# ihmcrobotics/mecano

Measured on AMD Instinct MI355X. Metric: robot-configs/sec (RNEA+ABA), 30-DoF humanoid batch=4096, higher is better.
Workload: dtype f64; 1 GPU; 30-DoF humanoid (SixDoF pelvis + 24 revolute), RNEA and ABA of every configuration per step, fp64, AoS [B][n] state; entry_point=mh_rnea_aba_f64, batch_per_gpu=4096, global_batch=4096, nq=31, nv=30, bodies=25, parallelism=dp1 (batch sharded, no data-path collective), kernel_variant=topo:b5c1e26c784c54fa, model_seed=43, state_seed=2342

## Files before the change

### mecano_amd/csrc/mh_api.hip

```cpp
#include "../../include/mecano_hip.h"
#include "mh_dfs_kernels.h"
#include "mh_split_kernels.h"
#include "mh_gravity_kernels.h"
#include "mh_response_kernels.h"
#include "mh_minv_kernels.h"

#include <dlfcn.h>
#include <spawn.h>
#include <sys/wait.h>
#include <unistd.h>
#include <cerrno>
extern char **environ;
#include <unistd.h>

#include <algorithm>
#include <functional>
#include <array>
#include <cmath>
#include <cstdarg>
#include <cstdio>
#include <cstdlib>
#include <cstring>
#include <map>
#include <deque>
// ... 332 lines not shown
   d.consts = sizeof(T) == 8 ? (const void *)m->d_consts64 : (const void *)m->d_consts32;
   d.prog = m->d_prog, d.n_events = (int)m->prog.size();
   d.rnea_stack = m->rnea_stack, d.aba_stack = m->aba_stack, d.aba_hand = m->aba_hand;
   return d;
}

template <class ARGS>
void set_root_acceleration(ARGS &A, const mh_options &o, const double *gravity)
{
   using T = decltype(A.gx);
   if (o.use_root_acceleration)
   {
      A.rax = (T)o.root_acceleration[0], A.ray = (T)o.root_acceleration[1], A.raz = (T)o.root_acceleration[2];
      A.gx = (T)-o.root_acceleration[3], A.gy = (T)-o.root_acceleration[4], A.gz = (T)-o.root_acceleration[5];
   }
   else
   {
      A.rax = T(0), A.ray = T(0), A.raz = T(0);
      A.gx = gravity ? (T)gravity[0] : T(0), A.gy = gravity ? (T)gravity[1] : T(0), A.gz = gravity ? (T)gravity[2] : T(0);
   }
}

mh_status check_common(mh_model_t &model, int64_t B, const mh_options *opts)
{
   if (!model)
      return fail(MH_ERR_INVALID_ARGUMENT, "model is NULL");
   if (opts && opts->context)
   {
      mh_model *c = ((mh_context *)opts->context)->m;
      if (c->parent != (model->parent ? model->parent : model))
         return fail(MH_ERR_INVALID_ARGUMENT, "opts->context belongs to another model");
      model = c;
   }
   if (B < 0)
      return fail(MH_ERR_BAD_DIMENSION, "negative batch size %lld", (long long)B);
   if (opts && opts->layout != MH_LAYOUT_AOS && opts->layout != MH_LAYOUT_SOA)
      return fail(MH_ERR_INVALID_ARGUMENT, "unknown layout %d", opts->layout);
   int cur = 0;
   if (hipGetDevice(&cur) != hipSuccess)
      return fail(MH_ERR_NO_DEVICE, "no usable HIP device");
   if (cur != model->device)
      return fail(MH_ERR_INVALID_ARGUMENT, "model lives on device %d but the calling thread's device is %d", model->device, cur);
   return MH_OK;
}
mh_status begin_call(mh_model_t &model, int64_t B, const mh_options *opts_in, mh_options &opts)
{
   if (opts_in)
      opts = *opts_in;
   else
      mh_options_default(&opts);
   return check_common(model, B, &opts);
}

long groups_of(int64_t B) { return (B + 63) / 64; }

void set_strides(long &bs, long &es, bool soa, int64_t B, long n) { bs = soa ? 1 : n, es = soa ? B : 1; }

template <typename T>
mh::Args<T> make_args(const mh_model *m, int64_t B, const mh_options &o)
{
   mh::Args<T> A{};
   A.m = dev_model<T>(m);
   A.B = B;
   const bool soa = o.layout == MH_LAYOUT_SOA;
   set_strides(A.q_bs, A.q_es, soa, B, m->nq);
   set_strides(A.v_bs, A.v_es, soa, B, m->nv);
   set_strides(A.f_bs, A.f_es, soa, B, (long)m->n * 6);
   return A;
}
template <typename T>
mh::Args<T> make_args(const mh_model *m, int64_t B, const mh_options &o, const double *gravity)
{
   mh::Args<T> A = make_args<T>(m, B, o);
   set_root_acceleration(A, o, gravity);
   A.coriolis = o.consider_coriolis, A.accel = o.consider_accelerations;
   return A;
}

bool spec_done(int rc, const char *what, mh_status &st)
{
   if (rc == (int)hipErrorNotSupported)
      return false;
   st = rc == 0 ? MH_OK : fail(MH_ERR_HIP, "%s: %s", what, hipGetErrorString((hipError_t)rc));
   return true;
}

mh_status raise_lds_limit(mh_model *model, const void *kern, size_t lds)
{
   if (lds > 64 * 1024 && model->lds_attr[kern] < lds)
   {
      HIP_TRY(hipFuncSetAttribute(kern, hipFuncAttributeMaxDynamicSharedMemorySize, (int)lds));
      model->lds_attr[kern] = lds;
   }
   return MH_OK;
}

bool auto_transpose(const mh_model *m, int64_t B) { return B >= 8192 && m->nq + m->nv >= 64; }
bool transposes(const mh_model *m, int64_t B) { return m->use_transpose >= 0 ? m->use_transpose != 0 : auto_transpose(m, B); }

int split_flags(const mh_model *m, int algo, bool soa)
{
   int flags = m->ident_maps ? SPEC_IDENT : 0;
   if (!soa && m->dense_maps && m->force_io != 0 && m->spec.split_lds_bytes(algo, SPEC_IO_LDS, m->nq, m->nv) <= 160 * 1024)
      flags |= SPEC_IO_LDS;
   return flags;
}
bool split_ok(const mh_model *m, int algo, int64_t B, bool soa)
{
   if (!m->spec.launch_split || !m->spec.split_usable || !m->spec.split_usable() || !m->use_spec || m->use_split == 0)
      return false;
   if (m->spec.split_lds_bytes(algo, split_flags(m, algo, soa), m->nq, m->nv) > 160 * 1024)
      return false;
   if (m->use_split == 1 || algo == 1 || algo == 0)
      return true;
   const long groups = groups_of(B);
   const long waves = groups * 4 * (algo == 2 ? 2 : 1);
   return waves <= (long)m->cu_count * 4 * kFusedFactor;
}

bool zv_ok(const mh_model *m, int64_t B, bool soa, int jobs)
{
   if (!m->spec.launch_zv || !m->spec.zv_usable || !m->spec.zv_usable() || !m->use_spec || !m->use_zv || m->use_split == 0)
      return false;
   if (soa || !m->dense_maps || m->force_io == 0 || m->n_locked > 0)
      return false;
   const long lds = m->spec.zv_lds_bytes(m->nq, m->nv);
   return lds > 0 && lds <= 160 * 1024 && (m->use_zv == 2 || groups_of(B) * jobs <= (long)m->cu_count);
}
std::mutex g_error_words_mutex;
std::vector<int *> g_error_words;
mh_status zv_check_error(mh_model *m)
{
   if (m->zv_error_host && *(volatile int *)m->zv_error_host != 0)
   {
      *(volatile int *)m->zv_error_host = 0;
      return fail(MH_ERR_HIP, "a bias-split forward dynamics launch gave up waiting for its bias rows (the accelerations of those configurations were written as NaN)");
   }
   return MH_OK;
}
mh_status check_all_error_words()
{
   std::lock_guard<std::mutex> lock(g_error_words_mutex);
   bool any = false;
   for (int *w : g_error_words)
      if (*(volatile int *)w != 0)
      {
         *(volatile int *)w = 0;
         any = true;
      }
   if (any)
      return fail(MH_ERR_HIP, "a bias-split forward dynamics launch gave up waiting for its bias rows (the accelerations of those configurations were written as NaN)");
   return MH_OK;
}
bool zv_self_signalling(const mh_model *m) { return m->ident_maps && m->spec.zv_self_signal && m->spec.zv_self_signal() != 0; }
mh_status zv_prepare(mh_model *m, int64_t B, hipStream_t stream)
{
   const size_t groups = (size_t)groups_of(B);
   mh_status st = ensure_bytes(m->zv_tau, groups * 64 * m->nv * sizeof(double));
   if (st != MH_OK)
      return st;
   if (zv_self_signalling(m) && m->zv_cols.bytes < groups * 64 * m->nv * sizeof(double))
   {
      st = ensure_bytes(m->zv_cols, std::max<size_t>(groups, 128) * 64 * m->nv * sizeof(double));
      if (st != MH_OK)
         return st;
      HIP_TRY(hipMemsetD32Async((hipDeviceptr_t)m->zv_cols.ptr, 0x7ff4a5a5, m->zv_cols.bytes / 4, stream));
   }
   if (m->zv_flags.bytes < groups * mh::ZV_SYNC_STRIDE * sizeof(int))
   {
      st = ensure_bytes(m->zv_flags, std::max<size_t>(groups, 1024) * mh::ZV_SYNC_STRIDE * sizeof(int));
      if (st != MH_OK)
         return st;
      HIP_TRY(hipMemsetAsync(m->zv_flags.ptr, 0, m->zv_flags.bytes, stream));
      m->zv_epoch = 0;
   }
   if (!m->zv_error_host)
   {
      HIP_TRY(hipHostMalloc((void **)&m->zv_error_host, 2 * sizeof(int), hipHostMallocMapped));
      m->zv_error_host[0] = m->zv_error_host[1] = 0;
      HIP_TRY(hipHostGetDevicePointer((void **)&m->zv_error_dev, m->zv_error_host, 0));
      std::lock_guard<std::mutex> lock(g_error_words_mutex);
      g_error_words.push_back(m->zv_error_host);
   }
   return MH_OK;
}
mh_status zv_launch(mh_model *m, mh::Args<double> &A, int jobs, hipStream_t stream, bool &done)
{
   done = false;
   mh_status st = zv_prepare(m, A.B, stream);
   if (st != MH_OK)
      return st;
   if (m->zv_epoch == 0x7fffffff)
   {
      HIP_TRY(hipDeviceSynchronize());
      HIP_TRY(hipMemsetAsync(m->zv_flags.ptr, 0, m->zv_flags.bytes, stream));
      m->zv_epoch = 0;
   }
   const bool self_signal = zv_self_signalling(m);
   if (self_signal && *(volatile int *)(m->zv_error_host + 1) != 0)
   {
      HIP_TRY(hipDeviceSynchronize());
      HIP_TRY(hipMemsetD32Async((hipDeviceptr_t)m->zv_cols.ptr, 0x7ff4a5a5, m->zv_cols.bytes / 4, stream));
      HIP_TRY(hipMemsetAsync(m->zv_flags.ptr, 0, m->zv_flags.bytes, stream));
      m->zv_epoch = 0;
      *(volatile int *)(m->zv_error_host + 1) = 0;
   }
   const int epoch = ++m->zv_epoch;
   int flags = SPEC_IO_LDS | (m->ident_maps ? SPEC_IDENT : 0);
   done = spec_done(m->spec.launch_zv(flags, &A, self_signal ? m->zv_cols.ptr : m->zv_tau.ptr, (int *)m->zv_flags.ptr, m->zv_error_dev, epoch, jobs,
                                      m->zv_same_l2, m->zv_wait_ticks, (void *)stream),
                    "bias-split kernel launch failed", st);
   return st;
}

bool zvb_ok(const mh_model *m, int64_t B, bool soa)
{
   if (!m->spec.launch_zvb || !m->spec.zvb_usable || !m->spec.zvb_usable() || !m->use_spec || !m->use_zvb || m->use_split == 0)
      return false;
   if (soa || !m->dense_maps || m->force_io == 0 || m->n_locked > 0)
      return false;
   return m->use_zvb == 2 || groups_of(B) >= 2 * (long)m->cu_count;
}
bool zvf_ok(const mh_model *m, int64_t B, bool soa)
{
   if (!m->spec.launch_zvf || !m->spec.zvf_usable || !m->spec.zvf_usable() || !m->use_spec || !m->use_zvf || m->use_split == 0)
      return false;
   if (soa || !m->dense_maps || !m->ident_maps || m->force_io == 0 || m->n_locked > 0)
      return false;
   return m->use_zvf == 2 || groups_of(B) > (long)m->cu_count;
}
bool rnea_ahead_ok(const mh_model *m, int64_t B, bool soa)
{
   if (!m->spec.launch_rnea_ahead || !m->spec.zvb_usable || !m->spec.zvb_usable() || !m->use_spec || !m->use_rnea_ahead || m->use_split == 0)
      return false;
   if (soa || !m->dense_maps || m->force_io == 0)
      return false;
   return m->use_rnea_ahead == 2 || groups_of(B) > 2 * (long)m->cu_count;
}
mh_status zvb_launch(mh_model *m, mh::Args<double> &A, hipStream_t stream, bool &done)
{
   done = false;
   const size_t padded = (size_t)(groups_of(A.B) * 64);
   mh_status st = ensure_bytes(m->zv_tau, (size_t)A.B * m->nv * sizeof(double));
   if (st == MH_OK)
      st = ensure_bytes(m->zvb_cs, std::max<size_t>(1, (size_t)m->spec.zvb_cs_rows()) * padded * sizeof(double));
   if (st != MH_OK)
      return st;
   const int flags = SPEC_IO_LDS | (m->ident_maps ? SPEC_IDENT : 0);
   const long groups = std::min<long>(groups_of(A.B), (long)m->cu_count * 2);
   done = spec_done(m->spec.launch_zvb(flags, &A, m->zv_tau.ptr, m->zvb_cs.ptr, (long)padded, (int)groups, m->zvb_which, (void *)stream),
                    "two-launch forward dynamics failed to launch", st);
   return st;
}

enum Algo
{
   ALGO_RNEA,
   ALGO_ABA,
   ALGO_CRBA
};

const mh_model::DfsPlan *dfs_plan(mh_model *m, int algo, int budget)
{
   if (m->parent)
      m = m->parent;
   std::lock_guard<std::mutex> lock(m->dfs_mutex);
   for (const mh_model::DfsPlan &p : m->dfs_plans)
      if (p.algo == algo && p.budget == budget)
         return &p;
   const int n = m->n;
   std::vector<int> meta = m->meta, frame(n), below(n, 0), lofs(n, 0), gofs(n, 0);
   std::vector<char> home(n, 0);
   auto MI = [&](int e, int k) -> int & { return meta[(size_t)e * mh::MI_STRIDE + k]; };
   for (int e = 0; e < n; e++)
      frame[e] = algo == 0 ? mh::rnea_frame_slots(MI(e, mh::MI_TYPE), MI(e, mh::MI_NCH))
                           : (algo == 1 ? mh::aba_frame_slots(MI(e, mh::MI_TYPE), MI(e, mh::MI_NCH)) : mh::pair_frame_slots(MI(e, mh::MI_TYPE), MI(e, mh::MI_NCH)));
   bool all_fit = true;
   {
      for (int e = n - 1; e >= 0; e--)
      {
         int need = below[e];
         if (frame[e] > 0 && below[e] + frame[e] <= budget)
            home[e] = 1, need += frame[e];
         else if (frame[e] > 0)
            all_fit = false;
         const int pe = MI(e, mh::MI_PARENT);
         if (pe >= 0)
            below[pe] = std::max(below[pe], need);
      }
   }
   if (!(m->dfs_place_greedy || (algo == 0 && budget < 64) || all_fit))
   {
      std::vector<int> worth(n, 0);
      std::vector<int> with_subtree(n, 0);
      for (int e = 0; e < n; e++)
         if (MI(e, mh::MI_PARENT) >= 0 && MI(e, mh::MI_NCH) > 0)
            with_subtree[MI(e, mh::MI_PARENT)]++;
      for (int e = 0; e < n; e++)
      {
         const int k = MI(e, mh::MI_NCH), jx = mh::jx_slots(MI(e, mh::MI_TYPE)), in_frame = std::max(0, with_subtree[e] - 1);
         if (k == 0)
            continue;
         if (algo == 0)
            worth[e] = k == 1 ? 2 * (6 + jx) : (6 + jx + 12) + (k - 1) * 12 + 6 + in_frame * 12 + (6 + jx);
         else
         {
            const int id = algo == 2 ? 6 : 0;
            const int acc = 27 + id;
            worth[e] = k == 1 ? 2 * (6 + jx) + 2 * id
                              : (12 + jx + 6 + id) + (k - 1) * (12 + id) + (in_frame > 0 ? acc + (in_frame - 1) * 2 * acc + acc : 0) + (12 + jx);
         }
      }
      const int W = budget + 1;
      std::vector<long> best((size_t)n * W, 0);
      std::vector<char> take((size_t)n * W, 0);
      std::vector<std::vector<int>> kids(n);
// ... 3309 lines not shown
```

### mecano_amd/csrc/mh_spec.hip

```cpp
#include "mh_spec_kernels.h"
#include "mh_zv_kernels.h"

#include <algorithm>
#include <atomic>
#include <cstdlib>
#include <type_traits>

#ifndef MH_SPEC_PART
#define MH_SPEC_PART 0
#endif
#ifndef MH_TOPO_N
#error "MH_TOPO_N / MH_TOPO_PARENTS / MH_TOPO_TYPES must be defined"
#endif

namespace
{
struct TP
{
   static constexpr int N = MH_TOPO_N;
   static constexpr int parent[N] = {MH_TOPO_PARENTS};
   static constexpr int type[N] = {MH_TOPO_TYPES};
};
constexpr int kParents[TP::N] = {MH_TOPO_PARENTS};
constexpr int kTypes[TP::N] = {MH_TOPO_TYPES};
// ... 73 lines not shown
      else
      {
         if (flags & F_ST_LDS)
            return go<ALGO, IO, ID, true>(A, grid, lds, s);
         return go<ALGO, IO, ID, false>(A, grid, lds, s);
      }
   }
   else
   {
      if constexpr (!kWholeTreeRnea)
         return hipErrorNotSupported;
      else
         return go<ALGO, IO, ID, false>(A, grid, lds, s);
   }
}
template <int ALGO>
hipError_t go_flags(int flags, const mh::Args<double> &A, int grid, size_t lds, hipStream_t s)
{
   const bool io = flags & F_IO_LDS, id = flags & F_IDENT;
   if (io && id)
      return go_st<ALGO, true, true>(flags, A, grid, lds, s);
   if (io)
      return go_st<ALGO, true, false>(flags, A, grid, lds, s);
   if (id)
      return go_st<ALGO, false, true>(flags, A, grid, lds, s);
   return go_st<ALGO, false, false>(flags, A, grid, lds, s);
}
}

template <bool ID>
hipError_t go_fused(const mh::Args<double> &A, int waves, hipStream_t stream)
{
   if constexpr (!kWholeTreeAba)
      return hipErrorNotSupported;
   else
   {
   auto kern = &mh::spec_fused_kernel<TP, double, ID>;
   const size_t lds = (size_t)std::max(lds_bytes(0, F_IO_LDS, A.m.nq, A.m.nv), lds_bytes(1, F_ST_LDS, A.m.nq, A.m.nv));
   static LdsAttr attr;
   if (const hipError_t e = ensure_lds_attr(reinterpret_cast<const void *>(kern), lds, attr); e != hipSuccess)
      return e;
   hipLaunchKernelGGL(kern, dim3(2 * waves), dim3(64), lds, stream, A);
   return hipGetLastError();
   }
}

using SPL = mh::Split<TP>;
static long split_lds_bytes(int algo, int flags, int nq, int nv)
{
   if (algo == 2)
      return std::max(split_lds_bytes(0, flags, nq, nv), split_lds_bytes(1, flags, nq, nv));
   long b = (long)(SPL::n_limbs() * (algo == 0 ? 6 : 27) + (algo == 1 ? SPL::TRUNK_SLOTS : SPL::RNEA_TRUNK_SLOTS)) * 64 * sizeof(double);
   if (flags & F_IO_LDS)
      b += (long)(nq + (algo == 1 ? 3 : 2) * nv) * 64 * sizeof(double);
   return b;
}
template <class K>
hipError_t launch_lds(K kern, const mh::Args<double> &A, int grid, size_t lds, LdsAttr &attr, hipStream_t stream)
{
   if (const hipError_t e = ensure_lds_attr(reinterpret_cast<const void *>(kern), lds, attr); e != hipSuccess)
      return e;
   hipLaunchKernelGGL(kern, dim3(grid), dim3(256), lds, stream, A);
   return hipGetLastError();
}
template <bool ID, bool IO>
hipError_t go_fused_split(const mh::Args<double> &A, int groups, hipStream_t stream)
{
   if constexpr (SPL::usable())
   {
      static LdsAttr attr_bytes;
      return launch_lds(&mh::spec_fused_split_kernel<TP, double, ID, IO>, A, 2 * groups,
                        (size_t)split_lds_bytes(2, IO ? F_IO_LDS : 0, A.m.nq, A.m.nv), attr_bytes, stream);
   }
   else
      return hipErrorNotSupported;
}
template <int ALGO, bool ID, bool IO>
hipError_t go_split(const mh::Args<double> &A, int groups, hipStream_t stream, bool occ3 = false)
{
   if constexpr (SPL::usable())
   {
      static LdsAttr attr_bytes, attr_occ3;
      if constexpr (ALGO == 0 && ID && !IO)
      {
         if (occ3)
            return launch_lds(&mh::spec_split_kernel_occ3<TP, double, ALGO, ID, IO>, A, groups,
                              (size_t)split_lds_bytes(ALGO, 0, A.m.nq, A.m.nv), attr_occ3, stream);
      }
      return launch_lds(&mh::spec_split_kernel<TP, double, ALGO, ID, IO>, A, groups,
                        (size_t)split_lds_bytes(ALGO, IO ? F_IO_LDS : 0, A.m.nq, A.m.nv), attr_bytes, stream);
   }
   else
      return hipErrorNotSupported;
}
template <bool ID, bool IO>
hipError_t go_split_algo(int algo, const mh::Args<double> &A, int groups, hipStream_t s, bool occ3)
{
   if (algo == 2)
      return go_fused_split<ID, IO>(A, groups, s);
   if (algo == 0)
      return go_split<0, ID, IO>(A, groups, s, occ3);
   if (algo == 1)
      return go_split<1, ID, IO>(A, groups, s);
   return hipErrorNotSupported;
}

extern "C" {
#if MH_SPEC_PART != 2
int mh_spec_split_usable(void) { return SPL::usable() ? 1 : 0; }
long mh_spec_split_lds_bytes(int algo, int flags, int nq, int nv) { return split_lds_bytes(algo, flags, nq, nv); }
int mh_spec_launch_split(int algo, int flags, const void *args, int groups, void *stream)
{
   const mh::Args<double> &A = *(const mh::Args<double> *)args;
   const bool id = flags & F_IDENT, io = flags & F_IO_LDS;
   hipStream_t s = (hipStream_t)stream;
   const bool occ3 = (flags & F_OCC3) != 0;
   if (flags & F_BODIES)
   {
#ifdef MH_SPEC_MINIMAL
      return (int)hipErrorNotSupported;
#else
      if constexpr (SPL::usable())
      {
         if (id && io && (algo == 0 || algo == 1))
         {
            static LdsAttr attr0, attr1;
            const size_t lds = (size_t)split_lds_bytes(algo, F_IO_LDS, A.m.nq, A.m.nv);
            if (algo == 0)
               return (int)launch_lds(&mh::spec_split_kernel<TP, double, 0, true, true, true>, A, groups, lds, attr0, s);
            return (int)launch_lds(&mh::spec_split_kernel<TP, double, 1, true, true, true>, A, groups, lds, attr1, s);
         }
      }
      return (int)hipErrorNotSupported;
#endif
   }
   if (id && io)
      return (int)go_split_algo<true, true>(algo, A, groups, s, occ3);
#ifdef MH_SPEC_MINIMAL
   return (int)hipErrorNotSupported;
#else
   if (id)
      return (int)go_split_algo<true, false>(algo, A, groups, s, occ3);
   if (io)
      return (int)go_split_algo<false, true>(algo, A, groups, s, occ3);
   return (int)go_split_algo<false, false>(algo, A, groups, s, occ3);
#endif
}
#endif
#if MH_SPEC_PART != 1
long mh_spec_zv_lds_bytes(int nq, int nv)
{
   if constexpr (!SPL::usable())
      return 0;
   const long inertia = (long)(SPL::n_limbs() * mh::ZV_XW + SPL::ZV_TRUNK_SLOTS + nq + 2 * nv) * 64 * (long)sizeof(double);
   return std::max(inertia, split_lds_bytes(0, F_IO_LDS, nq, nv) + (long)mh::zv_bias_extra_rows<TP>() * 64 * (long)sizeof(double));
}
int mh_spec_zv_usable(void) { return SPL::usable() ? 1 : 0; }
int mh_spec_zv_self_signal(void) { return MH_ZV_TWO_STAGE && MH_ZV_SELF_SIGNAL ? 1 : 0; }
#ifdef MH_ZV_PROBE
int mh_spec_zv_probe_read(void *dst, size_t bytes) { return (int)hipMemcpyFromSymbol(dst, HIP_SYMBOL(mh::zv_probe), bytes); }
int mh_spec_zv_probe_body_read(void *dst, size_t bytes) { return (int)hipMemcpyFromSymbol(dst, HIP_SYMBOL(mh::zv_probe_body), bytes); }
#endif
int mh_spec_launch_zv(int flags, const void *args, void *taup, int *sync_flags, int *error, int epoch, int jobs, int same_l2, unsigned wait_ticks, void *stream)
{
   if constexpr (SPL::usable())
   {
      const mh::Args<double> &A = *(const mh::Args<double> *)args;
      if (!(flags & F_IO_LDS) || (jobs != 2 && jobs != 3))
         return (int)hipErrorNotSupported;
      const size_t lds = (size_t)mh_spec_zv_lds_bytes(A.m.nq, A.m.nv);
      if (lds > 160 * 1024)
         return (int)hipErrorNotSupported;
      const long groups = (A.B + 63) / 64, padded = (groups + 7) / 8 * 8;
      const mh::ZvSync sy{sync_flags, error, epoch, jobs, same_l2 ? 1 : 0, wait_ticks};
      hipStream_t s = (hipStream_t)stream;
      if (A.q_next && (!(flags & F_IDENT) || jobs != 2 || !MH_ZV_TWO_STAGE))
         return (int)hipErrorNotSupported;
      if ((flags & F_IDENT) && A.q_next)
      {
         static LdsAttr attr_step;
         auto kern = &mh::spec_zv_kernel<TP, double, true, true>;
         if (const hipError_t e = ensure_lds_attr(reinterpret_cast<const void *>(kern), lds, attr_step); e != hipSuccess)
            return (int)e;
         hipLaunchKernelGGL(kern, dim3((unsigned)(padded * jobs)), dim3(256), lds, s, A.q, A.qd, A.in3b, A.B, jobs, A, (double *)taup, sy);
         return (int)hipGetLastError();
      }
      if (flags & F_IDENT)
      {
         static LdsAttr attr;
         auto kern = &mh::spec_zv_kernel<TP, double, true>;
         if (const hipError_t e = ensure_lds_attr(reinterpret_cast<const void *>(kern), lds, attr); e != hipSuccess)
            return (int)e;
         hipLaunchKernelGGL(kern, dim3((unsigned)(padded * jobs)), dim3(256), lds, s, A.q, A.qd, A.in3b, A.B, jobs, A, (double *)taup, sy);
         return (int)hipGetLastError();
      }
#ifdef MH_SPEC_MINIMAL
      return (int)hipErrorNotSupported;
#else
      static LdsAttr attr2;
      auto kern = &mh::spec_zv_kernel<TP, double, false>;
      if (const hipError_t e = ensure_lds_attr(reinterpret_cast<const void *>(kern), lds, attr2); e != hipSuccess)
         return (int)e;
      hipLaunchKernelGGL(kern, dim3((unsigned)(padded * jobs)), dim3(256), lds, s, A.q, A.qd, A.in3b, A.B, jobs, A, (double *)taup, sy);
      return (int)hipGetLastError();
#endif
   }
   else
      return (int)hipErrorNotSupported;
}
int mh_spec_zvb_usable(void)
{
   if constexpr (SPL::usable())
      return mh::ZvbPlan<TP>::lds_slots() * 64 * (long)sizeof(double) * 2 <= 160 * 1024 ? 1 : 0;
   else
      return 0;
}
int mh_spec_zvb_cs_rows(void) { return 2 * TR::n_revolute(); }
long mh_spec_zvb_lds_bytes(int which, int nq, int nv)
{
   if constexpr (SPL::usable())
      return (long)(which == 0 ? mh::ZvbPlan<TP>::bias_lds_slots(nq, nv) : mh::ZvbPlan<TP>::lds_slots()) * 64 * (long)sizeof(double);
   else
      return 0;
}
int mh_spec_launch_zvb(int flags, const void *args, void *taup, void *cs, long cs_stride, int groups, int which, void *stream)
{
   if constexpr (SPL::usable())
   {
      const mh::Args<double> &A = *(const mh::Args<double> *)args;
      if (!(flags & F_IO_LDS) || !mh_spec_zvb_usable() || cs_stride < (A.B + 63) / 64 * 64 || groups < 1)
         return (int)hipErrorNotSupported;
      const size_t lds0 = (size_t)mh_spec_zvb_lds_bytes(0, A.m.nq, A.m.nv), lds1 = (size_t)mh_spec_zvb_lds_bytes(1, A.m.nq, A.m.nv);
      if (lds0 > 160 * 1024)
         return (int)hipErrorNotSupported;
      hipStream_t s = (hipStream_t)stream;
      auto run = [&](auto ident) -> hipError_t {
         constexpr bool ID = decltype(ident)::value;
         static LdsAttr attr0, attr1;
         auto k0 = &mh::spec_zvb_bias_kernel<TP, double, ID>;
         auto k1 = &mh::spec_zvb_kernel<TP, double, ID>;
         if (which & 1)
         {
            if (const hipError_t e = ensure_lds_attr(reinterpret_cast<const void *>(k0), lds0, attr0); e != hipSuccess)
               return e;
            hipLaunchKernelGGL(k0, dim3((unsigned)groups), dim3(256), lds0, s, A, (double *)taup, (double *)cs, cs_stride);
            if (const hipError_t e = hipGetLastError(); e != hipSuccess)
               return e;
         }
         if (which & 2)
         {
            if (const hipError_t e = ensure_lds_attr(reinterpret_cast<const void *>(k1), lds1, attr1); e != hipSuccess)
               return e;
            hipLaunchKernelGGL(k1, dim3((unsigned)groups), dim3(256), lds1, s, A, (const double *)taup, (const double *)cs, cs_stride);
            if (const hipError_t e = hipGetLastError(); e != hipSuccess)
               return e;
         }
         return hipSuccess;
      };
      if (flags & F_IDENT)
         return (int)run(std::true_type{});
#ifdef MH_SPEC_MINIMAL
      return (int)hipErrorNotSupported;
#else
      return (int)run(std::false_type{});
#endif
   }
   else
      return (int)hipErrorNotSupported;
}
int mh_spec_launch_rnea_ahead(int flags, const void *args, int groups, void *stream)
{
   if constexpr (SPL::usable())
   {
      const mh::Args<double> &A = *(const mh::Args<double> *)args;
      if (!(flags & F_IO_LDS) || !mh_spec_zvb_usable() || groups < 1 || A.body_acc || A.body_twist || A.m.nq != TR::total_cfgs() || A.m.nv != TR::total_dofs())
         return (int)hipErrorNotSupported;
      const size_t lds = (size_t)mh_spec_zvb_lds_bytes(0, A.m.nq, A.m.nv);
      if (lds * 2 > 160 * 1024)
         return (int)hipErrorNotSupported;
      hipStream_t s = (hipStream_t)stream;
      auto run = [&](auto ident) -> hipError_t {
         constexpr bool ID = decltype(ident)::value;
         static LdsAttr attr;
         auto k = &mh::spec_zvb_bias_kernel<TP, double, ID, false>;
         if (const hipError_t e = ensure_lds_attr(reinterpret_cast<const void *>(k), lds, attr); e != hipSuccess)
            return e;
         hipLaunchKernelGGL(k, dim3((unsigned)groups), dim3(256), lds, s, A, A.out, (double *)nullptr, 0L);
         return hipGetLastError();
      };
      if (flags & F_IDENT)
         return (int)run(std::true_type{});
#ifdef MH_SPEC_MINIMAL
      return (int)hipErrorNotSupported;
#else
      return (int)run(std::false_type{});
#endif
   }
   else
      return (int)hipErrorNotSupported;
}
int mh_spec_zvf_usable(void)
{
   if constexpr (SPL::usable())
      return mh::ZvfPlan<TP>::usable() ? 1 : 0;
   else
      return 0;
}
long mh_spec_zvf_lds_bytes(void)
{
   if constexpr (SPL::usable())
      return (long)mh::ZvfPlan<TP>::lds_slots() * 64 * (long)sizeof(double);
   else
      return 0;
}
int mh_spec_launch_zvf(int flags, const void *args, int groups, void *stream)
{
   if constexpr (SPL::usable())
   {
      const mh::Args<double> &A = *(const mh::Args<double> *)args;
      if (!(flags & F_IO_LDS) || !(flags & F_IDENT) || !mh_spec_zvf_usable() || groups < 1 || A.m.nq != TR::total_cfgs() || A.m.nv != TR::total_dofs())
         return (int)hipErrorNotSupported;
      if (A.q_next)
      {
         if constexpr (mh::ZvfPlan<TP>::step_usable())
         {
            static LdsAttr attr_step;
            return (int)launch_lds(&mh::spec_zvf_kernel<TP, double, true, true>, A, groups, (size_t)mh_spec_zvf_lds_bytes(), attr_step, (hipStream_t)stream);
         }
         else
            return (int)hipErrorNotSupported;
      }
      if (A.in3b && A.outb)
      {
         if constexpr (mh::ZvfPlan<TP>::pair_usable())
         {
            static LdsAttr attr_pair;
            return (int)launch_lds(&mh::spec_zvf_kernel<TP, double, true, false, true>, A, groups, (size_t)mh_spec_zvf_lds_bytes(), attr_pair, (hipStream_t)stream);
         }
         else
            return (int)hipErrorNotSupported;
      }
      static LdsAttr attr;
      return (int)launch_lds(&mh::spec_zvf_kernel<TP, double, true>, A, groups, (size_t)mh_spec_zvf_lds_bytes(), attr, (hipStream_t)stream);
   }
   else
      return (int)hipErrorNotSupported;
}
int mh_spec_zvf_pair_usable(void)
{
// ... 197 lines not shown
```

### mecano_amd/csrc/mh_spec_kernels.h

```cpp
#pragma once
#include "mh_kernels.h"

#define MH_BODY_FENCE() __builtin_amdgcn_sched_barrier(0)

namespace mh
{
template <class TP>
struct Tree
{
   static constexpr int N = TP::N;
   static constexpr int ndof(int j) { return TP::type[j] == JT_SIXDOF ? 6 : (TP::type[j] == JT_FIXED ? 0 : 1); }
   static constexpr int ncfg(int j) { return TP::type[j] == JT_SIXDOF ? 7 : (TP::type[j] == JT_FIXED ? 0 : 1); }
   static constexpr int dof_ofs(int j)
   {
      int s = 0;
      for (int i = 0; i < j; i++)
         s += ndof(i);
      return s;
   }
   static constexpr int cfg_ofs(int j)
   {
      int s = 0;
      for (int i = 0; i < j; i++)
         s += ncfg(i);
// ... 641 lines not shown
   MH_DEV void out(int k, T v) const
   {
      if constexpr (OUTMODE == 1)
         v = in3(k) - v;
      if constexpr (IO_LDS && OUTMODE != 2)
         lo[di(k)] = v;
      else
         orow[di(k) * v_es] = v;
   }
};

template <typename T>
struct JQ
{
   T q[7];
};
template <int TYPE, int CO, class CX, typename T>
MH_DEV JQ<T> spec_joint_read(const CX &cx)
{
   JQ<T> r;
   if constexpr (TYPE == JT_REVOLUTE || TYPE == JT_PRISMATIC)
      r.q[0] = cx.q(CO);
   else if constexpr (TYPE == JT_SIXDOF)
      for (int k = 0; k < 7; k++)
         r.q[k] = cx.q(CO + k);
   return r;
}
template <int TYPE, typename T>
MH_DEV JX<T> spec_joint_from(const JQ<T> &r)
{
   JX<T> jx;
   jx.c = T(1), jx.s = T(0), jx.d = T(0);
   if constexpr (TYPE == JT_REVOLUTE)
      sincos_t(r.q[0], jx.s, jx.c);
   else if constexpr (TYPE == JT_PRISMATIC)
      jx.d = r.q[0];
   else if constexpr (TYPE == JT_SIXDOF)
   {
      jx.X.R = quat_to_R(r.q[0], r.q[1], r.q[2], r.q[3]);
      jx.X.p = V3<T>{r.q[4], r.q[5], r.q[6]};
   }
   return jx;
}
template <int TYPE, int CO, class CX, typename T>
MH_DEV JX<T> spec_joint(const CX &cx)
{
   return spec_joint_from<TYPE, T>(spec_joint_read<TYPE, CO, CX, T>(cx));
}
template <int TYPE, int DO, int WHICH, class CX, typename T>
MH_DEV SV<T> spec_vec(const CX &cx, bool enabled)
{
   SV<T> o{V3<T>{T(0), T(0), T(0)}, V3<T>{T(0), T(0), T(0)}};
   if (!enabled)
      return o;
   auto rd = [&](int k) { return WHICH == 0 ? cx.qd(k) : cx.in3(k); };
   if constexpr (TYPE == JT_REVOLUTE)
      o.a.z = rd(DO);
   else if constexpr (TYPE == JT_PRISMATIC)
      o.l.z = rd(DO);
   else if constexpr (TYPE == JT_SIXDOF)
   {
      o.a = V3<T>{rd(DO + 0), rd(DO + 1), rd(DO + 2)};
      o.l = V3<T>{rd(DO + 3), rd(DO + 4), rd(DO + 5)};
   }
   return o;
}
template <int TYPE, int DO, class CX, typename T>
MH_DEV void spec_write(const CX &cx, SV<T> w)
{
   if constexpr (TYPE == JT_REVOLUTE)
      cx.out(DO, w.a.z);
   else if constexpr (TYPE == JT_PRISMATIC)
      cx.out(DO, w.l.z);
   else if constexpr (TYPE == JT_SIXDOF)
   {
      cx.out(DO + 0, w.a.x), cx.out(DO + 1, w.a.y), cx.out(DO + 2, w.a.z);
      cx.out(DO + 3, w.l.x), cx.out(DO + 4, w.l.y), cx.out(DO + 5, w.l.z);
   }
}

template <class TP, int J, int K, class CX, typename T>
MH_DEV void zvf_tau_put1(const CX &cx, T v)
{
   using SP = typename CX::SPolicy;
   if constexpr (SP::root_in_regs(J))
      cx.st.lbase[(SP::root_tau_slot() + K) * 64] = v;
   else
      cx.st.template put<J, SP::tau_slot(J) + K>(v);
}
template <class TP, int J, int K, class CX, typename T>
MH_DEV T zvf_tau_get1(const CX &cx)
{
   using SP = typename CX::SPolicy;
   if constexpr (SP::root_in_regs(J))
      return cx.st.lbase[(SP::root_tau_slot() + K) * 64];
   else if constexpr (SP::late_body(J))
      return cx.st.lbase[(SP::late_tau_slot(J) + K) * 64];
   else
      return cx.st.template get<J, SP::tau_slot(J) + K>();
}
template <class TP, int J, class CX, typename T>
MH_DEV void zvf_put_tau(const CX &cx, const SV<T> &h)
{
   constexpr int TYPE = TP::type[J], DO = Tree<TP>::dof_ofs(J);
   if constexpr (TYPE == JT_REVOLUTE)
      zvf_tau_put1<TP, J, 0, CX, T>(cx, cx.in3(DO) - h.a.z);
   else if constexpr (TYPE == JT_PRISMATIC)
      zvf_tau_put1<TP, J, 0, CX, T>(cx, cx.in3(DO) - h.l.z);
   else if constexpr (TYPE == JT_SIXDOF)
   {
      zvf_tau_put1<TP, J, 0, CX, T>(cx, cx.in3(DO + 0) - h.a.x), zvf_tau_put1<TP, J, 1, CX, T>(cx, cx.in3(DO + 1) - h.a.y);
      zvf_tau_put1<TP, J, 2, CX, T>(cx, cx.in3(DO + 2) - h.a.z), zvf_tau_put1<TP, J, 3, CX, T>(cx, cx.in3(DO + 3) - h.l.x);
      zvf_tau_put1<TP, J, 4, CX, T>(cx, cx.in3(DO + 4) - h.l.y), zvf_tau_put1<TP, J, 5, CX, T>(cx, cx.in3(DO + 5) - h.l.z);
   }
}

template <int J, class CX, typename T>
MH_DEV void spec_body_outputs(const CX &cx, const SV<T> &acc, const SV<T> &twist)
{
   if constexpr (CX::bodies)
   {
      const CRef<T> c{cx.C + J * MC_STRIDE};
      const int ext = cx.meta[J * MI_STRIDE + MI_EXT];
      if (cx.bacc)
         store_body_motion<T>(c, cx.bacc, cx.f_es, ext, acc);
      if (cx.btw)
         store_body_motion<T>(c, cx.btw, cx.f_es, ext, twist);
   }
}

template <int LIMB, int XW, int I, class CX, typename T>
MH_DEV void x_put(const CX &cx, T v)
{
   cx.xbase[(LIMB * XW + I) * 64] = v;
}
template <int LIMB, int XW, int I, class CX, typename T>
MH_DEV T x_get(const CX &cx)
{
   return cx.xbase[(LIMB * XW + I) * 64];
}
template <int LIMB, int XW, int I0, class CX, typename T>
MH_DEV void x_put6(const CX &cx, const SV<T> &w)
{
   x_put<LIMB, XW, I0 + 0, CX, T>(cx, w.a.x), x_put<LIMB, XW, I0 + 1, CX, T>(cx, w.a.y), x_put<LIMB, XW, I0 + 2, CX, T>(cx, w.a.z);
   x_put<LIMB, XW, I0 + 3, CX, T>(cx, w.l.x), x_put<LIMB, XW, I0 + 4, CX, T>(cx, w.l.y), x_put<LIMB, XW, I0 + 5, CX, T>(cx, w.l.z);
}
template <int LIMB, int XW, int I0, class CX, typename T>
MH_DEV SV<T> x_get6(const CX &cx)
{
   return SV<T>{V3<T>{x_get<LIMB, XW, I0 + 0, CX, T>(cx), x_get<LIMB, XW, I0 + 1, CX, T>(cx), x_get<LIMB, XW, I0 + 2, CX, T>(cx)},
                V3<T>{x_get<LIMB, XW, I0 + 3, CX, T>(cx), x_get<LIMB, XW, I0 + 4, CX, T>(cx), x_get<LIMB, XW, I0 + 5, CX, T>(cx)}};
}

template <class TP, int J, typename T, class CX, int MODE = 0>
struct RneaSub
{
   template <int K>
   static MH_DEV void children(const CX &cx, const SV<T> &v, const SV<T> &a, SV<T> &f)
   {
      if constexpr (K < Tree<TP>::n_children(J))
      {
         constexpr int C = Tree<TP>::child(J, K);
         if constexpr (MODE == 1 && !Split<TP>::is_trunk(C))
            f = f + x_get6<Split<TP>::limb_index(C), 6, 0, CX, T>(cx);
         else
            f = f + RneaSub<TP, C, T, CX, MODE>::run(cx, v, a);
         children<K + 1>(cx, v, a, f);
      }
   }
   static MH_DEV SV<T> run(const CX &cx, const SV<T> &vp, const SV<T> &ap)
   {
      MH_BODY_FENCE();
      constexpr int TYPE = TP::type[J];
      constexpr int DO = Tree<TP>::dof_ofs(J), CO = Tree<TP>::cfg_ofs(J);
      const CRef<T> c{cx.C + J * MC_STRIDE};
      constexpr bool PRE3 = CX::csmode == 3 && MH_ZVF_PRE && TYPE == JT_REVOLUTE && Split<TP>::usable() && !Split<TP>::is_trunk(J);
      constexpr bool PRE = (CX::rnea_pre && TYPE == JT_REVOLUTE) || PRE3;
      constexpr int PS = PRE3 ? 7 : 0;
      JQ<T> jq;
      if constexpr (!PRE)
         jq = spec_joint_read<TYPE, CO, CX, T>(cx);
      const SV<T> vJ = spec_vec<TYPE, DO, 0, CX, T>(cx, cx.coriolis != 0);
      const SV<T> aJ = spec_vec<TYPE, DO, 1, CX, T>(cx, cx.accel != 0);
      const XF<T> Xb = load_xb_j<TP, J, T>(c);
      const RI<T> I = load_inertia<T>(c);
      MH_BODY_FENCE();
      JX<T> jx;
      if constexpr (PRE)
         jx.c = cx.st.template get<J, PS>(), jx.s = cx.st.template get<J, PS + 1>(), jx.d = T(0);
      else
         jx = spec_joint_from<TYPE, T>(jq);
      if constexpr (CX::csmode == 1 && TYPE == JT_REVOLUTE)
      {
         constexpr int R = Tree<TP>::rev_index(J);
         cx.cs[(2 * R) * cx.cs_stride] = jx.c, cx.cs[(2 * R + 1) * cx.cs_stride] = jx.s;
      }
      if constexpr (CX::csmode == 3 && TYPE == JT_REVOLUTE && !PRE3)
      {
         cx.st.template put<J, 7>(jx.c);
         cx.st.template put<J, 8>(jx.s);
      }
      const V3<T> Z{T(0), T(0), T(0)};
      SV<T> v = motion_down(TYPE, jx, Xb, vp) + vJ;
      const SV<T> a = motion_down(TYPE, jx, Xb, ap) + aJ + crm(v, vJ);
      if (!cx.coriolis)
         v = SV<T>{Z, Z};
      spec_body_outputs<J, CX, T>(cx, a, v);
      SV<T> f = mul(I, a) + crf(v, mul(I, v));
      if (cx.frow)
         f = f - load_fext<T>(c, cx.frow, cx.f_es, cx.meta[J * MI_STRIDE + MI_EXT]);
      MH_BODY_FENCE();
      children<0>(cx, v, a, f);
      MH_BODY_FENCE();
      if constexpr (CX::csmode == 3)
         zvf_put_tau<TP, J, CX, T>(cx, f);
      else
         spec_write<TYPE, DO, CX, T>(cx, f);
      const T *c2p = cx.C + J * MC_STRIDE;
      asm volatile("" : "+s"(c2p));
      const SV<T> up = force_up(TYPE, jx, load_xb_j<TP, J, T>(CRef<T>{c2p}), f);
      MH_BODY_FENCE();
      return up;
   }
};
template <class TP, typename T, class CX, int MODE = 0, int K = 0>
MH_DEV void rnea_roots(const CX &cx)
{
   if constexpr (K < Tree<TP>::n_children(-1))
   {
      const V3<T> Z{T(0), T(0), T(0)};
      (void)RneaSub<TP, Tree<TP>::child(-1, K), T, CX, MODE>::run(cx, SV<T>{Z, Z}, SV<T>{cx.a0a, cx.a0l});
      rnea_roots<TP, T, CX, MODE, K + 1>(cx);
   }
}
template <class CX, typename T>
MH_DEV lds_ptr<T> rnea_park(const CX &cx)
{
   if constexpr (CX::csmode == 3)
      return cx.park;
   else
      return cx.st.lbase;
}
template <class TP, int J, typename T, class CX, int FK = -1, int OWN = 0>
MH_DEV void trunk_va(const CX &cx, SV<T> &v, SV<T> &a)
{
   constexpr int TYPE = TP::type[J];
   constexpr int DO = Tree<TP>::dof_ofs(J), CO = Tree<TP>::cfg_ofs(J);
   const V3<T> Z{T(0), T(0), T(0)};
   SV<T> vp{Z, Z}, ap{cx.a0a, cx.a0l};
   if constexpr (TP::parent[J] >= 0)
      trunk_va<TP, TP::parent[J], T, CX, FK, OWN>(cx, vp, ap);
   MH_BODY_FENCE();
   const CRef<T> c{cx.C + J * MC_STRIDE};
   constexpr bool PRE = CX::rnea_pre && TYPE == JT_REVOLUTE;
   JQ<T> jq;
   if constexpr (!PRE)
      jq = spec_joint_read<TYPE, CO, CX, T>(cx);
   const SV<T> vJ = spec_vec<TYPE, DO, 0, CX, T>(cx, cx.coriolis != 0);
   const SV<T> aJ = spec_vec<TYPE, DO, 1, CX, T>(cx, cx.accel != 0);
   const XF<T> Xb = load_xb_j<TP, J, T>(c);
   MH_BODY_FENCE();
   JX<T> jx;
   if constexpr (PRE)
      jx.c = cx.st.template get<J, 0>(), jx.s = cx.st.template get<J, 1>(), jx.d = T(0);
   else
      jx = spec_joint_from<TYPE, T>(jq);
   v = motion_down(TYPE, jx, Xb, vp) + vJ;
   a = motion_down(TYPE, jx, Xb, ap) + aJ + crm(v, vJ);
   if (!cx.coriolis)
      v = SV<T>{Z, Z};
   if constexpr (FK >= 0 && Split<TP>::template f_limb_sel<OWN>(J) == FK)
   {
      spec_body_outputs<J, CX, T>(cx, a, v);
      const RI<T> I = load_inertia<T>(c);
      SV<T> f = mul(I, a) + crf(v, mul(I, v));
      if (cx.frow)
         f = f - load_fext<T>(c, cx.frow, cx.f_es, cx.meta[J * MI_STRIDE + MI_EXT]);
      constexpr int S0 = Split<TP>::rnea_trunk_slot(J);
      const lds_ptr<T> t = rnea_park<CX, T>(cx);
      t[(S0 + 0) * 64] = f.a.x, t[(S0 + 1) * 64] = f.a.y, t[(S0 + 2) * 64] = f.a.z;
      t[(S0 + 3) * 64] = f.l.x, t[(S0 + 4) * 64] = f.l.y, t[(S0 + 5) * 64] = f.l.z;
      t[(S0 + 6) * 64] = jx.c, t[(S0 + 7) * 64] = jx.s;
      if constexpr (CX::csmode == 1 && TYPE == JT_REVOLUTE)
      {
         constexpr int R = Tree<TP>::rev_index(J);
         cx.cs[(2 * R) * cx.cs_stride] = jx.c, cx.cs[(2 * R + 1) * cx.cs_stride] = jx.s;
      }
   }
   MH_BODY_FENCE();
}
template <class TP, int J, typename T, class CX>
struct RneaTrunkUp
{
   template <int K>
   static MH_DEV void children(const CX &cx, SV<T> &f)
   {
      if constexpr (K < Tree<TP>::n_children(J))
      {
         constexpr int C = Tree<TP>::child(J, K);
         if constexpr (!Split<TP>::is_trunk(C))
            f = f + x_get6<Split<TP>::limb_index(C), 6, 0, CX, T>(cx);
         else
            f = f + RneaTrunkUp<TP, C, T, CX>::run(cx);
         children<K + 1>(cx, f);
      }
   }
   static MH_DEV SV<T> run(const CX &cx)
   {
      MH_BODY_FENCE();
      constexpr int TYPE = TP::type[J];
      constexpr int DO = Tree<TP>::dof_ofs(J), CO = Tree<TP>::cfg_ofs(J), S0 = Split<TP>::rnea_trunk_slot(J);
      const lds_ptr<T> t = rnea_park<CX, T>(cx);
      SV<T> f{V3<T>{t[(S0 + 0) * 64], t[(S0 + 1) * 64], t[(S0 + 2) * 64]}, V3<T>{t[(S0 + 3) * 64], t[(S0 + 4) * 64], t[(S0 + 5) * 64]}};
      JX<T> jx;
      jx.c = t[(S0 + 6) * 64], jx.s = t[(S0 + 7) * 64], jx.d = T(0);
      if constexpr (TYPE != JT_REVOLUTE && TP::parent[J] >= 0)
         jx = spec_joint_from<TYPE, T>(spec_joint_read<TYPE, CO, CX, T>(cx));
      children<0>(cx, f);
      MH_BODY_FENCE();
      if constexpr (CX::csmode == 3)
      {
         zvf_put_tau<TP, J, CX, T>(cx, f);
         if constexpr (TYPE == JT_REVOLUTE)
         {
            cx.st.template put<J, 7>(jx.c);
            cx.st.template put<J, 8>(jx.s);
         }
      }
      else
         spec_write<TYPE, DO, CX, T>(cx, f);
      SV<T> up = f;
      if constexpr (TP::parent[J] >= 0)
         up = force_up(TYPE, jx, load_xb_j<TP, J, T>(CRef<T>{cx.C + J * MC_STRIDE}), f);
      MH_BODY_FENCE();
      return up;
   }
};
template <class TP, typename T, class CX, int K = 0>
MH_DEV void rnea_trunk_roots(const CX &cx)
{
   if constexpr (K < Tree<TP>::n_children(-1))
   {
      (void)RneaTrunkUp<TP, Tree<TP>::child(-1, K), T, CX>::run(cx);
      rnea_trunk_roots<TP, T, CX, K + 1>(cx);
   }
}
template <class TP, int J, typename T, class CX>
MH_DEV SV<T> trunk_v(const CX &cx)
{
   constexpr int TYPE = TP::type[J];
   constexpr int DO = Tree<TP>::dof_ofs(J), CO = Tree<TP>::cfg_ofs(J);
   const V3<T> Z{T(0), T(0), T(0)};
   SV<T> vp{Z, Z};
   if constexpr (TP::parent[J] >= 0)
      vp = trunk_v<TP, TP::parent[J], T, CX>(cx);
   MH_BODY_FENCE();
   const CRef<T> c{cx.C + J * MC_STRIDE};
   const JQ<T> jq = spec_joint_read<TYPE, CO, CX, T>(cx);
   const SV<T> vJ = spec_vec<TYPE, DO, 0, CX, T>(cx, true);
   const XF<T> Xb = load_xb_j<TP, J, T>(c);
   MH_BODY_FENCE();
   const JX<T> jx = spec_joint_from<TYPE, T>(jq);
   const SV<T> v = motion_down(TYPE, jx, Xb, vp) + vJ;
   MH_BODY_FENCE();
   return v;
}

template <typename T>
struct AbaUp
{
   ABI<T> I;
   SV<T> p;
};
template <typename T>
MH_DEV AbaUp<T> aba_up_zero()
{
   AbaUp<T> z;
   z.I.A = S3<T>{T(0), T(0), T(0), T(0), T(0), T(0)};
   z.I.L = z.I.A;
   z.I.C = M3<T>{T(0), T(0), T(0), T(0), T(0), T(0), T(0), T(0), T(0)};
   z.p = SV<T>{V3<T>{T(0), T(0), T(0)}, V3<T>{T(0), T(0), T(0)}};
   return z;
}

template <int LIMB, class CX, typename T>
MH_DEV void x_put_up(const CX &cx, const AbaUp<T> &u)
{
   constexpr int XW = 27;
   x_put<LIMB, XW, 0, CX, T>(cx, u.I.A.xx), x_put<LIMB, XW, 1, CX, T>(cx, u.I.A.xy), x_put<LIMB, XW, 2, CX, T>(cx, u.I.A.xz);
   x_put<LIMB, XW, 3, CX, T>(cx, u.I.A.yy), x_put<LIMB, XW, 4, CX, T>(cx, u.I.A.yz), x_put<LIMB, XW, 5, CX, T>(cx, u.I.A.zz);
   x_put<LIMB, XW, 6, CX, T>(cx, u.I.L.xx), x_put<LIMB, XW, 7, CX, T>(cx, u.I.L.xy), x_put<LIMB, XW, 8, CX, T>(cx, u.I.L.xz);
   x_put<LIMB, XW, 9, CX, T>(cx, u.I.L.yy), x_put<LIMB, XW, 10, CX, T>(cx, u.I.L.yz), x_put<LIMB, XW, 11, CX, T>(cx, u.I.L.zz);
   x_put<LIMB, XW, 12, CX, T>(cx, u.I.C.xx), x_put<LIMB, XW, 13, CX, T>(cx, u.I.C.xy), x_put<LIMB, XW, 14, CX, T>(cx, u.I.C.xz);
   x_put<LIMB, XW, 15, CX, T>(cx, u.I.C.yx), x_put<LIMB, XW, 16, CX, T>(cx, u.I.C.yy), x_put<LIMB, XW, 17, CX, T>(cx, u.I.C.yz);
   x_put<LIMB, XW, 18, CX, T>(cx, u.I.C.zx), x_put<LIMB, XW, 19, CX, T>(cx, u.I.C.zy), x_put<LIMB, XW, 20, CX, T>(cx, u.I.C.zz);
   x_put6<LIMB, XW, 21, CX, T>(cx, u.p);
}
template <int LIMB, class CX, typename T>
MH_DEV AbaUp<T> x_get_up(const CX &cx)
{
   constexpr int XW = 27;
   AbaUp<T> u;
   u.I.A = S3<T>{x_get<LIMB, XW, 0, CX, T>(cx), x_get<LIMB, XW, 1, CX, T>(cx), x_get<LIMB, XW, 2, CX, T>(cx),
                 x_get<LIMB, XW, 3, CX, T>(cx), x_get<LIMB, XW, 4, CX, T>(cx), x_get<LIMB, XW, 5, CX, T>(cx)};
   u.I.L = S3<T>{x_get<LIMB, XW, 6, CX, T>(cx), x_get<LIMB, XW, 7, CX, T>(cx), x_get<LIMB, XW, 8, CX, T>(cx),
                 x_get<LIMB, XW, 9, CX, T>(cx), x_get<LIMB, XW, 10, CX, T>(cx), x_get<LIMB, XW, 11, CX, T>(cx)};
   u.I.C = M3<T>{x_get<LIMB, XW, 12, CX, T>(cx), x_get<LIMB, XW, 13, CX, T>(cx), x_get<LIMB, XW, 14, CX, T>(cx),
                 x_get<LIMB, XW, 15, CX, T>(cx), x_get<LIMB, XW, 16, CX, T>(cx), x_get<LIMB, XW, 17, CX, T>(cx),
                 x_get<LIMB, XW, 18, CX, T>(cx), x_get<LIMB, XW, 19, CX, T>(cx), x_get<LIMB, XW, 20, CX, T>(cx)};
   u.p = x_get6<LIMB, XW, 21, CX, T>(cx);
   return u;
}

template <class TP, int J, typename T, class CX, int MODE = 0>
struct AbaIn
{
   template <int K>
   static MH_DEV void children(const CX &cx, const SV<T> &v, AbaUp<T> &acc)
   {
      if constexpr (K < Tree<TP>::n_children(J))
      {
         constexpr int C = Tree<TP>::child(J, K);
         AbaUp<T> c;
         if constexpr ((MODE == 1 || MODE == 2) && !Split<TP>::is_trunk(C))
            c = x_get_up<Split<TP>::limb_index(C), CX, T>(cx);
         else if constexpr (MODE == 2)
            c = x_get_up<Split<TP>::sub_slot(C), CX, T>(cx);
         else
            c = AbaIn<TP, C, T, CX, MODE>::run(cx, v);
         if constexpr (K == 0)
            acc = c;
         else
         {
            add(acc.I, c.I);
            acc.p = acc.p + c.p;
// ... 872 lines not shown
}
template <class TP, typename T, class CX>
MH_DEV void rnea_pre_all(const CX &cx)
{
   if constexpr (CX::rnea_pre)
   {
      bool bad = false;
      rnea_pre_all_bodies<TP, true, 0, T, CX>(cx, bad);
      if (__builtin_expect(bad, 0))
         rnea_pre_all_bodies<TP, false, 0, T, CX>(cx, bad);
   }
}
template <class TP, typename T, int ALGO, bool IO_LDS, bool IDENT, bool ST_LDS>
MH_DEV void spec_wave(const Args<T> &A, long wave, long nwaves, lds_ptr<T> lds)
{
   using CX = Ctx<T, IO_LDS, IDENT, std::conditional_t<ALGO == 0 && MH_RNEA_PRE != 0, RneaPreStore<TP>, WholeStore<TP, ST_LDS ? ST_LDS_KIND : ST_GLOBAL_KIND>>>;
   const int nq = A.m.nq, nv = A.m.nv;
   const lds_ptr<T> lq = lds, lqd = lq + (IO_LDS ? 64 * nq : 0), lx = lqd + (IO_LDS ? 64 * nv : 0), lst = lx + (IO_LDS ? 64 * nv : 0);
   warm_scalar_cache(A.m.consts, A.m.n * MC_STRIDE * (int)sizeof(T));
   if constexpr (!IDENT)
   {
      warm_scalar_cache(A.m.dof_map, nv * 4);
      warm_scalar_cache(A.m.cfg_map, nq * 4);
   }
#ifdef MH_PROBE
#define MH_WSTAMP(k)                                                                                                                       \
   do                                                                                                                                      \
   {                                                                                                                                       \
      const unsigned long long t_ = __builtin_amdgcn_s_memrealtime();                                                                      \
      if (threadIdx.x == 0)                                                                                                                \
         ((unsigned long long *)(A.out + A.B * nv))[(cfg0 / 64) * 32 + (k)] = t_;                                                          \
   } while (0)
#else
#define MH_WSTAMP(k)
#endif
   for (long cfg0 = wave * 64; cfg0 < A.B; cfg0 += nwaves * 64)
   {
      const int rows = (int)(A.B - cfg0 < 64 ? A.B - cfg0 : 64);
      MH_WSTAMP(0);
      if constexpr (IO_LDS)
      {
         wave_stage_in<T, Tree<TP>::total_cfgs(), Tree<TP>::total_dofs()>(lq, lqd, lx, A.q + cfg0 * nq, A.qd + cfg0 * nv, A.in3 + cfg0 * nv, rows);
         __syncthreads();
      }
      MH_WSTAMP(1);
      if ((int)threadIdx.x < rows)
      {
         CX cx;
         fill_ctx<T>(cx, A, cfg0 + threadIdx.x);
         cx.lq = lq + threadIdx.x * nq, cx.lqd = lqd + threadIdx.x * nv, cx.lx = lx + threadIdx.x * nv;
         cx.lo = cx.lx;
         cx.wave = 0, cx.xbase = lst;
         cx.st.lbase = lst + threadIdx.x;
         cx.st.gbase = A.ws;
         cx.st.stride = A.ws_stride, cx.st.lane = wave * 64 + threadIdx.x;
         asm volatile("" : "+v"(cx.st.lane));
         if constexpr (ALGO == 0)
         {
            rnea_pre_all<TP, T, CX>(cx);
            rnea_roots<TP, T, CX>(cx);
         }
         else
         {
            aba_roots_in<TP, T, CX>(cx);
            MH_WSTAMP(4);
            asm volatile("" ::: "memory");
            asm volatile("" : "+v"(cx.qrow), "+v"(cx.qdrow), "+v"(cx.lq), "+v"(cx.lqd), "+v"(cx.st.lbase), "+v"(cx.st.lane));
            aba_roots_out<TP, T, CX>(cx);
         }
      }
      MH_WSTAMP(2);
      if constexpr (IO_LDS)
      {
         __syncthreads();
         wave_copy_out<T>(A.out + cfg0 * nv, lx, rows * nv);
         __syncthreads();
      }
      MH_WSTAMP(3);
   }
}

template <class TP, typename T, int ALGO, bool IO_LDS, bool IDENT, bool ST_LDS>
__global__ void __launch_bounds__(64) spec_kernel(Args<T> A)
{
   extern __shared__ double lds_raw[];
   spec_wave<TP, T, ALGO, IO_LDS, IDENT, ST_LDS>(A, blockIdx.x, gridDim.x, (lds_ptr<T>)lds_raw);
}

template <class TP, typename T, bool IDENT>
__global__ void __launch_bounds__(64) spec_fused_kernel(Args<T> A)
{
   extern __shared__ double lds_raw[];
   const long half = gridDim.x / 2;
   if ((long)blockIdx.x < half)
      spec_wave<TP, T, 0, true, IDENT, false>(A, blockIdx.x, half, (lds_ptr<T>)lds_raw);
   else
   {
      Args<T> A2 = A;
      A2.in3 = A.in3b, A2.out = A.outb;
      spec_wave<TP, T, 1, false, IDENT, true>(A2, blockIdx.x - half, half, (lds_ptr<T>)lds_raw);
   }
}

template <class TP, int W, int OWN, bool FAST, int J, typename T, class CX>
MH_DEV void rnea_pre_bodies(const CX &cx, bool &bad)
{
   if constexpr (J < TP::N)
   {
      constexpr int PS = CX::rnea_pre ? 0 : 7;
      if constexpr (TP::type[J] == JT_REVOLUTE && RneaPreSet<TP, OWN>::evaluates(W, J) && (CX::rnea_pre || !Split<TP>::is_trunk(J)))
      {
         const T x = cx.q(Tree<TP>::cfg_ofs(J));
         T s, c;
         if constexpr (FAST)
         {
            sincos_fast(x, s, c);
            bad = bad || !sincos_in_fast_range(x);
         }
         else
            sincos_t(x, s, c);
         cx.st.template put<J, PS>(c);
         cx.st.template put<J, PS + 1>(s);
      }
      rnea_pre_bodies<TP, W, OWN, FAST, J + 1, T, CX>(cx, bad);
   }
}
template <class TP, int W, int OWN, typename T, class CX>
MH_DEV void rnea_pre_pass(const CX &cx)
{
   if constexpr (CX::rnea_pre || (CX::csmode == 3 && MH_ZVF_PRE))
   {
      bool bad = false;
      rnea_pre_bodies<TP, W, OWN, true, 0, T, CX>(cx, bad);
      if (__builtin_expect(bad, 0))
         rnea_pre_bodies<TP, W, OWN, false, 0, T, CX>(cx, bad);
   }
}
template <class TP, int W, int K, int PC, typename T, class CX, int OWN = 0>
MH_DEV void split_rnea_limbs_of(const CX &cx, SV<T> &vp, SV<T> &ap)
{
   using S = Split<TP>;
   if constexpr (K < S::n_limbs())
   {
      if constexpr (S::template owner_sel<OWN>(K) == W)
      {
         constexpr int R = S::limb_root(K), P = TP::parent[R];
         if constexpr (P != PC)
         {
            const V3<T> Z{T(0), T(0), T(0)};
            vp = SV<T>{Z, Z}, ap = SV<T>{cx.a0a, cx.a0l};
            if constexpr (P >= 0)
               trunk_va<TP, P, T, CX, K, OWN>(cx, vp, ap);
         }
         x_put6<K, 6, 0, CX, T>(cx, RneaSub<TP, R, T, CX, 0>::run(cx, vp, ap));
         split_rnea_limbs_of<TP, W, K + 1, P, T, CX, OWN>(cx, vp, ap);
      }
      else
         split_rnea_limbs_of<TP, W, K + 1, PC, T, CX, OWN>(cx, vp, ap);
   }
}
template <class TP, int W, int K, int PC, typename T, class CX>
MH_DEV void split_aba_limbs_of(const CX &cx, SV<T> &vp)
{
   using S = Split<TP>;
   if constexpr (K < S::n_limbs())
   {
      if constexpr (S::owner(K) == W)
      {
         constexpr int R = S::limb_root(K), P = TP::parent[R];
         if constexpr (P != PC)
         {
            const V3<T> Z{T(0), T(0), T(0)};
            vp = SV<T>{Z, Z};
            if constexpr (P >= 0)
               vp = trunk_v<TP, P, T, CX>(cx);
         }
         x_put_up<K, CX, T>(cx, AbaIn<TP, R, T, CX, 0>::run(cx, vp));
         split_aba_limbs_of<TP, W, K + 1, P, T, CX>(cx, vp);
      }
      else
         split_aba_limbs_of<TP, W, K + 1, PC, T, CX>(cx, vp);
   }
}
template <class TP, int W, typename T, class CX, int OWN = 0>
MH_DEV void split_rnea_limbs(const CX &cx)
{
   if constexpr (W < 4)
   {
      if (cx.wave == W)
      {
         rnea_pre_pass<TP, W, OWN, T, CX>(cx);
         const V3<T> Z{T(0), T(0), T(0)};
         SV<T> vp{Z, Z}, ap{Z, Z};
         split_rnea_limbs_of<TP, W, 0, -2, T, CX, OWN>(cx, vp, ap);
      }
      else
         split_rnea_limbs<TP, W + 1, T, CX, OWN>(cx);
   }
}
template <class TP, int W, typename T, class CX>
MH_DEV void split_aba_limbs(const CX &cx)
{
   if constexpr (W < 4)
   {
      if (cx.wave == W)
      {
         const V3<T> Z{T(0), T(0), T(0)};
         SV<T> vp{Z, Z};
         split_aba_limbs_of<TP, W, 0, -2, T, CX>(cx, vp);
      }
      else
         split_aba_limbs<TP, W + 1, T, CX>(cx);
   }
}

template <class TP, int W, int K, int PC, int LATE, typename T, class CX>
MH_DEV void staged_limbs_of(const CX &cx, SV<T> &vp)
{
   using S = Split<TP>;
   if constexpr (K < S::n_limbs())
   {
      if constexpr (S::owner(K) == W && (S::is_late(K) ? 1 : 0) == LATE)
      {
         constexpr int R = S::limb_root(K), P = TP::parent[R];
         if constexpr (P != PC)
         {
            const V3<T> Z{T(0), T(0), T(0)};
            vp = SV<T>{Z, Z};
            if constexpr (P >= 0)
               vp = trunk_v<TP, P, T, CX>(cx);
         }
         x_put_up<K, CX, T>(cx, AbaIn<TP, R, T, CX, (S::cut_limb(W) == K ? 3 : 0)>::run(cx, vp));
         staged_limbs_of<TP, W, K + 1, P, LATE, T, CX>(cx, vp);
      }
      else
         staged_limbs_of<TP, W, K + 1, PC, LATE, T, CX>(cx, vp);
   }
}
template <class TP, int W, int I, typename T, class CX>
MH_DEV void staged_subtrunks_of(const CX &cx)
{
   using S = Split<TP>;
   if constexpr (I < S::n_sub())
   {
      constexpr int ST = S::sub_top(I);
      if constexpr (S::sub_owner(ST) == W)
      {
         const SV<T> vr = trunk_v<TP, S::root(), T, CX>(cx);
         x_put_up<S::sub_slot(ST), CX, T>(cx, AbaIn<TP, ST, T, CX, 1>::run(cx, vr));
      }
      staged_subtrunks_of<TP, W, I + 1, T, CX>(cx);
   }
}
template <class TP, int W, typename T, class CX>
MH_DEV void split_aba_staged(const CX &cx)
{
   using S = Split<TP>;
   if constexpr (W < 4)
   {
      if (cx.wave == W)
      {
         const V3<T> Z{T(0), T(0), T(0)};
         SV<T> vp{Z, Z};
         staged_limbs_of<TP, W, 0, -2, 0, T, CX>(cx, vp);
         if constexpr (S::cut_limb(W) < 0)
            __syncthreads();
         staged_limbs_of<TP, W, 0, -2, 1, T, CX>(cx, vp);
         staged_subtrunks_of<TP, W, 0, T, CX>(cx);
      }
      else
         split_aba_staged<TP, W + 1, T, CX>(cx);
   }
}

template <class TP, int J, typename T>
MH_DEV void integrate_rows(int wave, lds_ptr<T> q, lds_ptr<T> v, lds_ptr<T> a, T dt, T hdd)
{
   using TR = Tree<TP>;
   if constexpr (J < TP::N)
   {
      if ((J & 3) == wave)
      {
         constexpr int TYPE = TP::type[J], D0 = TR::dof_ofs(J), C0 = TR::cfg_ofs(J);
         if constexpr (TYPE == JT_REVOLUTE || TYPE == JT_PRISMATIC)
         {
            const T q0 = q[C0], v0 = v[D0], a0 = a[D0];
            q[C0] = hdd * a0 + dt * v0 + q0;
            v[D0] = dt * a0 + v0;
         }
         else if constexpr (TYPE == JT_SIXDOF)
         {
            T qx = q[C0], qy = q[C0 + 1], qz = q[C0 + 2], qs = q[C0 + 3];
            V3<T> p{q[C0 + 4], q[C0 + 5], q[C0 + 6]}, w{v[D0], v[D0 + 1], v[D0 + 2]}, vl{v[D0 + 3], v[D0 + 4], v[D0 + 5]};
            const V3<T> al{a[D0], a[D0 + 1], a[D0 + 2]}, ac{a[D0 + 3], a[D0 + 4], a[D0 + 5]};
            integrate_sixdof<T>(dt, hdd, qx, qy, qz, qs, p, w, vl, al, ac, nullptr);
            q[C0] = qx, q[C0 + 1] = qy, q[C0 + 2] = qz, q[C0 + 3] = qs, q[C0 + 4] = p.x, q[C0 + 5] = p.y, q[C0 + 6] = p.z;
            v[D0] = w.x, v[D0 + 1] = w.y, v[D0 + 2] = w.z, v[D0 + 3] = vl.x, v[D0 + 4] = vl.y, v[D0 + 5] = vl.z;
         }
      }
      integrate_rows<TP, J + 1, T>(wave, q, v, a, dt, hdd);
   }
}

template <class TP, typename T, int ALGO, bool IDENT, bool IO_LDS, bool BODIES = false>
MH_DEV void split_group(const Args<T> &A, long group, long ngroups, lds_ptr<T> lds)
{
   using S = Split<TP>;
// ... 487 lines not shown
```

### mecano_amd/csrc/mh_zv_kernels.h

```cpp
#pragma once
#include "mh_spec_kernels.h"

namespace mh
{
template <class TP>
struct ZvStore
{
   static constexpr int REG_SLOTS = Split<TP>::zv_reg_slots();
   static constexpr int kind(int j) { return Split<TP>::is_trunk(j) ? ST_LDS_KIND : ST_REG_KIND; }
   static constexpr int index(int j) { return Split<TP>::is_trunk(j) ? Split<TP>::zv_trunk_slot(j) : Split<TP>::zv_reg_slot(j); }
   static constexpr bool shared(int j) { return !Split<TP>::is_trunk(j); }
};
template <class TP>
struct ZvbStore
{
   using S = Split<TP>;
   static constexpr bool root_in_regs(int j) { return S::staged() && j == S::root(); }
   static constexpr int REG_SLOTS = S::zv_reg_slots() + (S::staged() ? Tree<TP>::zv_slots_of(S::root() < 0 ? 0 : S::root(), true) : 0);
   static constexpr int trunk_slot(int j)
   {
      int s = 0;
      for (int i = 0; i < j; i++)
         s += S::is_trunk(i) && !root_in_regs(i) ? Tree<TP>::zv_slots_of(i, false) : 0;
      return s;
   }
   static constexpr int TRUNK_SLOTS = trunk_slot(TP::N);
   static constexpr int kind(int j) { return S::is_trunk(j) && !root_in_regs(j) ? ST_LDS_KIND : ST_REG_KIND; }
   static constexpr int index(int j) { return root_in_regs(j) ? S::zv_reg_slots() : (S::is_trunk(j) ? trunk_slot(j) : S::zv_reg_slot(j)); }
   static constexpr bool shared(int j) { return kind(j) == ST_REG_KIND; }
};
template <class TP>
struct ZvfPlan;
template <class TP>
struct ZvfStore
{
   using S = Split<TP>;
   using TR = Tree<TP>;
   static constexpr bool slot_homes = true;
   static constexpr bool mailed(int j) { return ZvfPlan<TP>::use_mail() && !S::is_trunk(j) && S::limb_index_of_body(j) == S::mailed_limb(); }
   static constexpr int slot_kind(int j, int k) { return mailed(j) && k >= 7 ? ST_LDS_KIND : kind(j); }
   static constexpr int slot_index(int j, int k) { return mailed(j) && k >= 7 ? ZvfPlan<TP>::mail_base() + (k - 7) : index(j) + k; }
   static constexpr bool root_in_regs(int j) { return S::staged() && j == S::root(); }
   static constexpr int limb_slots(int j) { return TR::zv_slots_of(j, true) + TR::ndof(j); }
   static constexpr int reg_slot(int j)
   {
      int s = 0;
      for (int i = 0; i < j; i++)
         s += !S::is_trunk(i) && S::owner(S::limb_index_of_body(i)) == S::owner(S::limb_index_of_body(j)) ? limb_slots(i) : 0;
      return s;
   }
   static constexpr int limb_reg_slots()
   {
      int best = 0;
      for (int w = 0; w < 4; w++)
      {
         int n = 0;
         for (int j = 0; j < TP::N; j++)
            n += !S::is_trunk(j) && S::owner(S::limb_index_of_body(j)) == w ? limb_slots(j) : 0;
         best = n > best ? n : best;
      }
      return best;
   }
   static constexpr int REG_SLOTS = limb_reg_slots() + (S::staged() ? TR::zv_slots_of(S::root() < 0 ? 0 : S::root(), true) : 0);
   static constexpr int trunk_slot(int j)
   {
      int s = 0;
      for (int i = 0; i < j; i++)
         s += S::is_trunk(i) && !root_in_regs(i) ? TR::zv_slots_of(i, false) + TR::ndof(i) : 0;
      return s;
   }
   static constexpr int root_tau_slot() { return trunk_slot(TP::N); }
   static constexpr int ROOT_TAU_SLOTS = S::staged() ? TR::ndof(S::root() < 0 ? 0 : S::root()) : 0;
   static constexpr bool owns_late(int w)
   {
      for (int k = 0; k < S::n_limbs(); k++)
         if (S::is_late(k) && S::owner(k) == w)
            return true;
      return false;
   }
   static constexpr bool late_body(int j) { return S::staged() && !S::is_trunk(j) && owns_late(S::owner(S::limb_index_of_body(j))); }
   static constexpr int late_tau_slot(int j)
   {
      int s = trunk_slot(TP::N) + ROOT_TAU_SLOTS;
      for (int i = 0; i < j; i++)
         s += late_body(i) ? TR::ndof(i) : 0;
      return s;
   }
   static constexpr int TRUNK_SLOTS = late_tau_slot(TP::N);
   static constexpr int tau_slot(int j) { return TR::zv_slots_of(j, !S::is_trunk(j)); }
   static constexpr int kind(int j) { return S::is_trunk(j) && !root_in_regs(j) ? ST_LDS_KIND : ST_REG_KIND; }
   static constexpr int index(int j) { return root_in_regs(j) ? limb_reg_slots() : (S::is_trunk(j) ? trunk_slot(j) : reg_slot(j)); }
   static constexpr bool shared(int j) { return kind(j) == ST_REG_KIND; }
};
#ifdef MH_ZV_PROBE
__device__ unsigned long long zv_probe[4096 * 3 * 4 * 16];
#define ZV_STAMP(job, ph)                                                                                                                  \
   do                                                                                                                                      \
   {                                                                                                                                       \
      const unsigned long long t_ = __builtin_amdgcn_s_memrealtime();                                                                      \
      if ((threadIdx.x & 63) == 0 && k < 4096)                                                                                             \
         zv_probe[((k * 3 + (job)) * 4 + (threadIdx.x >> 6)) * 16 + (ph)] = t_;                                                            \
   } while (0)
__device__ unsigned long long zv_probe_body[4096 * 32 * 4];
#ifdef MH_ZV_PROBE_BODY
#define ZV_STAMP_BODY(body, ph)                                                                                                            \
   do                                                                                                                                      \
   {                                                                                                                                       \
      const unsigned long long t_ = __builtin_amdgcn_s_memrealtime();                                                                      \
      if ((threadIdx.x & 63) == 0 && cx.own < 4096 && ((body) != 0 || cx.wave == 0))                                                      \
         zv_probe_body[(cx.own * 32 + (body)) * 4 + (ph)] = t_;                                                                            \
   } while (0)
#else
#define ZV_STAMP_BODY(body, ph)
#endif
#else
#define ZV_STAMP(job, ph)
#define ZV_STAMP_BODY(body, ph)
#endif
MH_DEV void zv_lds_barrier()
{
   asm volatile("s_waitcnt lgkmcnt(0)\n\ts_barrier" ::: "memory");
}
template <class CX>
MH_DEV void zv_fold_barrier()
{
   zv_lds_barrier();
}
constexpr int ZV_XW = 21;

template <int LIMB, class CX, typename T>
MH_DEV void x_put_ia(const CX &cx, const ABI<T> &I)
{
   constexpr int XW = ZV_XW;
   x_put<LIMB, XW, 0, CX, T>(cx, I.A.xx), x_put<LIMB, XW, 1, CX, T>(cx, I.A.xy), x_put<LIMB, XW, 2, CX, T>(cx, I.A.xz);
   x_put<LIMB, XW, 3, CX, T>(cx, I.A.yy), x_put<LIMB, XW, 4, CX, T>(cx, I.A.yz), x_put<LIMB, XW, 5, CX, T>(cx, I.A.zz);
   x_put<LIMB, XW, 6, CX, T>(cx, I.L.xx), x_put<LIMB, XW, 7, CX, T>(cx, I.L.xy), x_put<LIMB, XW, 8, CX, T>(cx, I.L.xz);
   x_put<LIMB, XW, 9, CX, T>(cx, I.L.yy), x_put<LIMB, XW, 10, CX, T>(cx, I.L.yz), x_put<LIMB, XW, 11, CX, T>(cx, I.L.zz);
   x_put<LIMB, XW, 12, CX, T>(cx, I.C.xx), x_put<LIMB, XW, 13, CX, T>(cx, I.C.xy), x_put<LIMB, XW, 14, CX, T>(cx, I.C.xz);
   x_put<LIMB, XW, 15, CX, T>(cx, I.C.yx), x_put<LIMB, XW, 16, CX, T>(cx, I.C.yy), x_put<LIMB, XW, 17, CX, T>(cx, I.C.yz);
   x_put<LIMB, XW, 18, CX, T>(cx, I.C.zx), x_put<LIMB, XW, 19, CX, T>(cx, I.C.zy), x_put<LIMB, XW, 20, CX, T>(cx, I.C.zz);
}
template <int LIMB, class CX, typename T>
MH_DEV ABI<T> x_get_ia(const CX &cx)
{
   constexpr int XW = ZV_XW;
   ABI<T> I;
   I.A = S3<T>{x_get<LIMB, XW, 0, CX, T>(cx), x_get<LIMB, XW, 1, CX, T>(cx), x_get<LIMB, XW, 2, CX, T>(cx),
               x_get<LIMB, XW, 3, CX, T>(cx), x_get<LIMB, XW, 4, CX, T>(cx), x_get<LIMB, XW, 5, CX, T>(cx)};
   I.L = S3<T>{x_get<LIMB, XW, 6, CX, T>(cx), x_get<LIMB, XW, 7, CX, T>(cx), x_get<LIMB, XW, 8, CX, T>(cx),
               x_get<LIMB, XW, 9, CX, T>(cx), x_get<LIMB, XW, 10, CX, T>(cx), x_get<LIMB, XW, 11, CX, T>(cx)};
   I.C = M3<T>{x_get<LIMB, XW, 12, CX, T>(cx), x_get<LIMB, XW, 13, CX, T>(cx), x_get<LIMB, XW, 14, CX, T>(cx),
               x_get<LIMB, XW, 15, CX, T>(cx), x_get<LIMB, XW, 16, CX, T>(cx), x_get<LIMB, XW, 17, CX, T>(cx),
               x_get<LIMB, XW, 18, CX, T>(cx), x_get<LIMB, XW, 19, CX, T>(cx), x_get<LIMB, XW, 20, CX, T>(cx)};
   return I;
}
template <typename T>
MH_DEV ABI<T> abi_zero()
{
   ABI<T> z;
   z.A = S3<T>{T(0), T(0), T(0), T(0), T(0), T(0)};
   z.L = z.A;
   z.C = M3<T>{T(0), T(0), T(0), T(0), T(0), T(0), T(0), T(0), T(0)};
   return z;
}
// ... 113 lines not shown
            cx.st.template put<J, 8>(jx.s);
         }
      }
   }
};
template <class TP, int W, int I, typename T, class CX, bool FAST = false>
MH_DEV void zv_pre_subtrunks_of(const CX &cx, bool &bad)
{
   using S = Split<TP>;
   if constexpr (I < S::n_sub())
   {
      if constexpr (S::sub_owner(S::sub_top(I)) == W)
         ZvPreTrunk<TP, S::sub_top(I), T, CX, FAST>::run(cx, bad);
      zv_pre_subtrunks_of<TP, W, I + 1, T, CX, FAST>(cx, bad);
   }
}
#ifndef MH_ZV_PRE_WAVE
#define MH_ZV_PRE_WAVE 1
#endif
template <class TP, int W, int K, typename T, class CX, bool FAST>
MH_DEV void zv_pre_limbs_of(const CX &cx, bool &bad)
{
   using S = Split<TP>;
   if constexpr (K < S::n_limbs())
   {
      if constexpr (S::owner(K) == W)
         ZvPre<TP, S::limb_root(K), T, CX, FAST>::run(cx, bad);
      zv_pre_limbs_of<TP, W, K + 1, T, CX, FAST>(cx, bad);
   }
}
template <class TP, int W, typename T, class CX>
MH_DEV void zv_pre_wave(const CX &cx)
{
   using S = Split<TP>;
   bool bad = false;
   zv_pre_limbs_of<TP, W, 0, T, CX, true>(cx, bad);
   if constexpr (S::staged())
      zv_pre_subtrunks_of<TP, W, 0, T, CX, true>(cx, bad);
   if (__builtin_expect(bad, 0))
   {
      zv_pre_limbs_of<TP, W, 0, T, CX, false>(cx, bad);
      if constexpr (S::staged())
         zv_pre_subtrunks_of<TP, W, 0, T, CX, false>(cx, bad);
   }
}
template <class TP, int J, typename T, class CX, int MODE = 0>
struct ZvIn
{
   template <int K>
   static MH_DEV void children(const CX &cx, ABI<T> &acc)
   {
      if constexpr (K < Tree<TP>::n_children(J))
      {
         constexpr int C = Tree<TP>::child(J, K);
         ABI<T> c;
         if constexpr ((MODE == 1 || MODE == 2) && !Split<TP>::is_trunk(C))
            c = x_get_ia<Split<TP>::limb_index(C), CX, T>(cx);
         else if constexpr (MODE == 2)
            c = x_get_ia<Split<TP>::sub_slot(C), CX, T>(cx);
         else
            c = ZvIn<TP, C, T, CX, MODE>::run(cx);
         if constexpr (K == 0)
            acc = c;
         else
            add(acc, c);
         children<K + 1>(cx, acc);
      }
   }
   static MH_DEV ABI<T> run(const CX &cx)
   {
      MH_BODY_FENCE();
      constexpr int TYPE = TP::type[J];
      constexpr bool HAS_PARENT = TP::parent[J] >= 0;
      constexpr bool LEAF = Tree<TP>::n_children(J) == 0;
      constexpr int CO = Tree<TP>::cfg_ofs(J);
      ABI<T> up = abi_zero<T>();
      if constexpr (!LEAF)
         children<0>(cx, up);
      if constexpr (MODE == 3 && Split<TP>::is_cut(J))
         __syncthreads();
      MH_BODY_FENCE();
      ZV_STAMP_BODY(J, 0);
      const T *cp = cx.C + J * MC_STRIDE;
      asm volatile("" : "+s"(cp));
      const CRef<T> c{cp};
      constexpr bool PRE = TYPE == JT_REVOLUTE && ((!Split<TP>::is_trunk(J) && (MODE == 0 || MODE == 3)) || ((CX::csmode == 2 || (CX::csmode == 0 && MH_ZV_PRE_WAVE)) && Split<TP>::staged() && Split<TP>::is_trunk(J) && MODE == 1) || (CX::csmode == 3 && Split<TP>::is_trunk(J)));
      JQ<T> jq;
      JX<T> jx;
      if constexpr (TYPE == JT_REVOLUTE && CX::csmode == 2 && !PRE)
         jx = zv_revolute_joint<TP, J, CX, T>(cx);
      else if constexpr (!PRE)
         jq = spec_joint_read<TYPE, CO, CX, T>(cx);
      const RI<T> I = load_inertia<T>(c);
      MH_BODY_FENCE();
      ABI<T> IA = abi_from_rigid(I);
      if constexpr (!LEAF)
         add(IA, up);
      MH_BODY_FENCE();
      ZV_STAMP_BODY(J, 1);
      const XF<T> Xb = load_xb_j<TP, J, T>(c);
      if constexpr (PRE)
         jx.c = cx.st.template get<J, 7>(), jx.s = cx.st.template get<J, 8>(), jx.d = T(0);
      else if constexpr (!(TYPE == JT_REVOLUTE && CX::csmode == 2))
         jx = spec_joint_from<TYPE, T>(jq);
      ABI<T> out = abi_zero<T>();
      if constexpr (TYPE == JT_REVOLUTE || TYPE == JT_PRISMATIC)
      {
         V3<T> ua, ul;
         T D;
         if constexpr (TYPE == JT_REVOLUTE)
            ua = V3<T>{IA.A.xz, IA.A.yz, IA.A.zz}, ul = V3<T>{IA.C.zx, IA.C.zy, IA.C.zz}, D = IA.A.zz;
         else
            ua = V3<T>{IA.C.xz, IA.C.yz, IA.C.zz}, ul = V3<T>{IA.L.xz, IA.L.yz, IA.L.zz}, D = IA.L.zz;
         const T dinv = rcp_fast(D);
         const V3<T> sa = dinv * ua, sl = dinv * ul;
         cx.st.template put<J, 0>(sa.x), cx.st.template put<J, 1>(sa.y), cx.st.template put<J, 2>(sa.z);
         cx.st.template put<J, 3>(sl.x), cx.st.template put<J, 4>(sl.y), cx.st.template put<J, 5>(sl.z);
         cx.st.template put<J, 6>(dinv);
         if constexpr (TYPE == JT_REVOLUTE)
         {
            cx.st.template put<J, 7>(jx.c);
            cx.st.template put<J, 8>(jx.s);
         }
         if constexpr (HAS_PARENT)
         {
            if constexpr (TYPE == JT_REVOLUTE)
               rank1_down_revolute(IA, ua, ul, dinv);
            else
               rank1_down(IA, ua, ul, dinv);
#ifdef MH_ZV_PROBE_BODY
            MH_BODY_FENCE();
            ZV_STAMP_BODY(J, 2);
#endif
            abi_up(TYPE, jx, Xb, IA);
            out = IA;
         }
      }
      else if constexpr (TYPE == JT_SIXDOF)
         st_put_ldl<J, 0, CX, T>(cx, spd6_factor(IA));
      else if constexpr (HAS_PARENT)
      {
         abi_up(TYPE, jx, Xb, IA);
         out = IA;
      }
      MH_BODY_FENCE();
      ZV_STAMP_BODY(J, 3);
      return out;
   }
};

template <class TP, int J, typename T, class CX, int MODE = 0>
struct ZvFold
{
   template <int K>
   static MH_DEV void children(const CX &cx, SV<T> &pA)
   {
      if constexpr (K < Tree<TP>::n_children(J))
      {
         constexpr int C = Tree<TP>::child(J, K);
         SV<T> c;
         if constexpr ((MODE == 1 || MODE == 2) && !Split<TP>::is_trunk(C))
            c = x_get6<Split<TP>::limb_index(C), CX::fold_xw, 0, CX, T>(cx);
         else if constexpr (MODE == 2)
            c = x_get6<Split<TP>::sub_slot(C), CX::fold_xw, 6, CX, T>(cx);
         else
            c = ZvFold<TP, C, T, CX, MODE>::run(cx);
         if constexpr (K == 0)
            pA = c;
         else
            pA = pA + c;
         children<K + 1>(cx, pA);
      }
   }
   static MH_DEV SV<T> run(const CX &cx)
   {
      MH_BODY_FENCE();
      constexpr int TYPE = TP::type[J];
      constexpr bool HAS_PARENT = TP::parent[J] >= 0;
      constexpr bool LEAF = Tree<TP>::n_children(J) == 0;
      constexpr int DO = Tree<TP>::dof_ofs(J), CO = Tree<TP>::cfg_ofs(J);
      constexpr int RS = Tree<TP>::zv_result_slot(J, CX::SPolicy::shared(J));
      const V3<T> Z{T(0), T(0), T(0)};
      SV<T> pA{Z, Z};
      if constexpr (!LEAF)
         children<0>(cx, pA);
      MH_BODY_FENCE();
      const T *cp = cx.C + J * MC_STRIDE;
      asm volatile("" : "+s"(cp));
      const CRef<T> c{cp};
      SV<T> up{Z, Z};
      if constexpr (TYPE == JT_REVOLUTE || TYPE == JT_PRISMATIC)
      {
         T tau;
         if constexpr (CX::csmode == 3)
            tau = zvf_tau_get1<TP, J, 0, CX, T>(cx);
         else
            tau = cx.in3(DO);
         JX<T> jx;
         jx.c = T(1), jx.s = T(0), jx.d = T(0);
         if constexpr (TYPE == JT_REVOLUTE)
            jx.c = cx.st.template get<J, 7>(), jx.s = cx.st.template get<J, 8>();
         else if constexpr (HAS_PARENT)
            jx.d = cx.q(CO);
         const V3<T> sa{cx.st.template get<J, 0>(), cx.st.template get<J, 1>(), cx.st.template get<J, 2>()};
         const V3<T> sl{cx.st.template get<J, 3>(), cx.st.template get<J, 4>(), cx.st.template get<J, 5>()};
         const T dinv = cx.st.template get<J, 6>();
         const T u = tau - (TYPE == JT_REVOLUTE ? pA.a.z : pA.l.z);
         cx.st.template put<J, RS>(u * dinv);
         if constexpr (HAS_PARENT)
         {
            const XF<T> Xb = load_xb_j<TP, J, T>(c);
            const SV<T> pa = pA + SV<T>{u * sa, u * sl};
            up = force_up(TYPE, jx, Xb, pa);
         }
      }
      else if constexpr (TYPE == JT_SIXDOF)
      {
         SV<T> tau;
         if constexpr (CX::csmode == 3)
            tau = SV<T>{V3<T>{zvf_tau_get1<TP, J, 0, CX, T>(cx), zvf_tau_get1<TP, J, 1, CX, T>(cx), zvf_tau_get1<TP, J, 2, CX, T>(cx)},
                        V3<T>{zvf_tau_get1<TP, J, 3, CX, T>(cx), zvf_tau_get1<TP, J, 4, CX, T>(cx), zvf_tau_get1<TP, J, 5, CX, T>(cx)}};
         else
            tau = spec_vec<TYPE, DO, 1, CX, T>(cx, true);
         const SV<T> x = spd6_solve(st_get_ldl<J, CX, T>(cx), tau - pA);
         cx.st.template put<J, RS + 0>(x.a.x), cx.st.template put<J, RS + 1>(x.a.y), cx.st.template put<J, RS + 2>(x.a.z);
         cx.st.template put<J, RS + 3>(x.l.x), cx.st.template put<J, RS + 4>(x.l.y), cx.st.template put<J, RS + 5>(x.l.z);
         if constexpr (HAS_PARENT)
         {
            const JX<T> jx = spec_joint<TYPE, CO, CX, T>(cx);
            up = force_up(TYPE, jx, load_xb_j<TP, J, T>(c), tau);
         }
      }
      else if constexpr (HAS_PARENT)
      {
         JX<T> jx;
         jx.c = T(1), jx.s = T(0), jx.d = T(0);
         up = force_up(TYPE, jx, load_xb_j<TP, J, T>(c), pA);
      }
      MH_BODY_FENCE();
      return up;
   }
};

template <class TP, int J, typename T, class CX, int MODE = 0>
struct ZvOut
{
   template <int K>
   static MH_DEV void children(const CX &cx, const SV<T> &a)
   {
      if constexpr (K < Tree<TP>::n_children(J))
      {
         constexpr int C = Tree<TP>::child(J, K);
         if constexpr (MODE == 1 && !Split<TP>::is_trunk(C))
         {
            if (cx.wave == Split<TP>::owner(Split<TP>::limb_index(C)))
               ZvOut<TP, C, T, CX, 0>::run(cx, a);
         }
         else
            ZvOut<TP, C, T, CX, MODE>::run(cx, a);
         children<K + 1>(cx, a);
      }
   }
   static MH_DEV void run(const CX &cx, const SV<T> &ap)
   {
      MH_BODY_FENCE();
      constexpr int TYPE = TP::type[J];
      constexpr bool HAS_PARENT = TP::parent[J] >= 0;
      constexpr bool LEAF = Tree<TP>::n_children(J) == 0;
      constexpr int DO = Tree<TP>::dof_ofs(J), CO = Tree<TP>::cfg_ofs(J);
      constexpr int RS = Tree<TP>::zv_result_slot(J, CX::SPolicy::shared(J));
      const T *cp = cx.C + J * MC_STRIDE;
      asm volatile("" : "+s"(cp));
      const CRef<T> c{cp};
      const V3<T> Z{T(0), T(0), T(0)};
      SV<T> a{Z, Z};
      if constexpr (HAS_PARENT)
      {
         JX<T> jx;
         jx.c = T(1), jx.s = T(0), jx.d = T(0);
         if constexpr (TYPE == JT_REVOLUTE)
            jx.c = cx.st.template get<J, 7>(), jx.s = cx.st.template get<J, 8>();
         else if constexpr (TYPE != JT_FIXED)
            jx = spec_joint<TYPE, CO, CX, T>(cx);
         a = motion_down(TYPE, jx, load_xb_j<TP, J, T>(c), ap);
      }
      if constexpr (TYPE == JT_REVOLUTE || TYPE == JT_PRISMATIC)
      {
         const V3<T> sa{cx.st.template get<J, 0>(), cx.st.template get<J, 1>(), cx.st.template get<J, 2>()};
         const V3<T> sl{cx.st.template get<J, 3>(), cx.st.template get<J, 4>(), cx.st.template get<J, 5>()};
         const T qdd = cx.st.template get<J, RS>() - (dot(sa, a.a) + dot(sl, a.l));
         if (MODE == 0 || cx.wave == 0)
            cx.out(DO, qdd);
         if constexpr (TYPE == JT_REVOLUTE)
            a.a.z += qdd;
         else
            a.l.z += qdd;
      }
      else if constexpr (TYPE == JT_SIXDOF)
      {
         const SV<T> x{V3<T>{cx.st.template get<J, RS + 0>(), cx.st.template get<J, RS + 1>(), cx.st.template get<J, RS + 2>()},
                       V3<T>{cx.st.template get<J, RS + 3>(), cx.st.template get<J, RS + 4>(), cx.st.template get<J, RS + 5>()}};
         if (MODE == 0 || cx.wave == 0)
            spec_write<TYPE, DO, CX, T>(cx, x - a);
         a = x;
      }
      MH_BODY_FENCE();
      if constexpr (!LEAF)
         children<0>(cx, a);
   }
};

template <class TP, typename T, class CX, int MODE, int K = 0>
MH_DEV void zv_roots_in(const CX &cx)
{
   if constexpr (K < Tree<TP>::n_children(-1))
   {
      (void)ZvIn<TP, Tree<TP>::child(-1, K), T, CX, MODE>::run(cx);
      zv_roots_in<TP, T, CX, MODE, K + 1>(cx);
   }
}
template <class TP, typename T, class CX, int K = 0>
MH_DEV void zv_roots_fold(const CX &cx)
{
   if constexpr (K < Tree<TP>::n_children(-1))
   {
      (void)ZvFold<TP, Tree<TP>::child(-1, K), T, CX, 1>::run(cx);
      zv_roots_fold<TP, T, CX, K + 1>(cx);
   }
}
template <class TP, typename T, class CX, int K = 0>
MH_DEV void zv_roots_out(const CX &cx)
{
   if constexpr (K < Tree<TP>::n_children(-1))
   {
      const V3<T> Z{T(0), T(0), T(0)};
      ZvOut<TP, Tree<TP>::child(-1, K), T, CX, 1>::run(cx, SV<T>{Z, Z});
// ... 223 lines not shown
   using S = Split<TP>;
   if constexpr (I < S::n_sub())
   {
      constexpr int ST = S::sub_top(I);
      if constexpr (S::sub_owner(ST) == W)
         x_put6<S::sub_slot(ST), CX::fold_xw, 6, CX, T>(cx, ZvFold<TP, ST, T, CX, 1>::run(cx));
      zv_subtrunks_fold_of<TP, W, I + 1, T, CX>(cx);
   }
}
struct ZvNoHook
{
   MH_DEV void after_early() const {}
   MH_DEV void after_late() const {}
   MH_DEV void before_out() const {}
};
template <class TP, int W, typename T, class CX, class HOOK = ZvNoHook>
MH_DEV void zv_fold_out(const CX &cx, const HOOK &hook = HOOK())
{
   using S = Split<TP>;
   if constexpr (W < 4)
   {
      if (cx.wave == W)
      {
         if constexpr (S::staged())
         {
#ifdef MH_ZV_PROBE
            const long k = (long)cx.own;
#endif
            zv_limbs_fold_sel<TP, W, 0, 0, T, CX>(cx);
            hook.after_early();
            ZV_STAMP(1, 7);
            zv_fold_barrier<CX>();
            zv_limbs_fold_sel<TP, W, 0, 1, T, CX>(cx);
            hook.after_late();
            zv_subtrunks_fold_of<TP, W, 0, T, CX>(cx);
            ZV_STAMP(1, 8);
            zv_fold_barrier<CX>();
            (void)ZvFold<TP, S::root(), T, CX, 2>::run(cx);
            ZV_STAMP(1, 9);
         }
         else
         {
            zv_limbs_fold_sel<TP, W, 0, -1, T, CX>(cx);
            hook.after_early();
            zv_fold_barrier<CX>();
            hook.after_late();
            zv_roots_fold<TP, T, CX>(cx);
         }
         if constexpr (CX::csmode >= 2)
            zv_fold_barrier<CX>();
         hook.before_out();
         asm volatile("" ::: "memory");
         zv_roots_out_wave<TP, W, T, CX>(cx);
      }
      else
         zv_fold_out<TP, W + 1, T, CX, HOOK>(cx, hook);
   }
}

template <typename T, int N, int NT>
MH_DEV void zv_stage_rows(lds_ptr<T> dst, const T *src, int rows)
{
   constexpr int U = (64 * N + NT - 1) / NT;
   T r[U];
   const int n = rows * N, t = threadIdx.x;
#pragma unroll
   for (int u = 0; u < U; u++)
      r[u] = t + NT * u < n ? src[t + NT * u] : T(0);
#pragma unroll
   for (int u = 0; u < U; u++)
      if (t + NT * u < 64 * N)
         dst[t + NT * u] = r[u];
}

struct ZvSync
{
   int *flags;
   int *error;
   int epoch;
   int jobs;
   int same_l2;
   unsigned wait_ticks;
};
MH_DEV int zv_xcc_id() { return (int)(__builtin_amdgcn_s_getreg((31 << 11) | 20) & 0xf); }
MH_DEV int zv_mail_key(int epoch, int xcc) { return (int)(((unsigned)epoch & 0x03ffffffu) << 5) | 16 | xcc; }

MH_DEV bool zv_wait(const ZvSync &sy, long k)
{
   const int *f = sy.flags + k * ZV_SYNC_STRIDE;
   if (__hip_atomic_load(f, __ATOMIC_RELAXED, __HIP_MEMORY_SCOPE_AGENT) == sy.epoch)
      return true;
   const unsigned long long t0 = __builtin_amdgcn_s_memrealtime();
   for (;;)
   {
      __builtin_amdgcn_s_sleep(1);
      if (__hip_atomic_load(f, __ATOMIC_RELAXED, __HIP_MEMORY_SCOPE_AGENT) == sy.epoch)
         return true;
      if (__builtin_amdgcn_s_memrealtime() - t0 > (unsigned long long)sy.wait_ticks)
      {
         if ((threadIdx.x & 63) == 0)
            __hip_atomic_store(sy.error, 1, __ATOMIC_RELAXED, __HIP_MEMORY_SCOPE_SYSTEM);
         return false;
      }
   }
}
template <typename T, int NT>
MH_DEV void zv_publish_rows(T *dst, lds_ptr<T> src, int n, bool same_l2)
{
   if (same_l2)
      for (int i = threadIdx.x; i < n; i += NT)
         __hip_atomic_store(dst + i, src[i], __ATOMIC_RELAXED, __HIP_MEMORY_SCOPE_WORKGROUP);
   else
      for (int i = threadIdx.x; i < n; i += NT)
         __hip_atomic_store(dst + i, src[i], __ATOMIC_RELAXED, __HIP_MEMORY_SCOPE_AGENT);
}
template <typename T, int N, int NT>
MH_DEV void zv_fetch_rows(lds_ptr<T> dst, const T *src, int rows)
{
   constexpr int U = (64 * N + NT - 1) / NT;
   T r[U];
   const int n = rows * N, t = threadIdx.x;
#pragma unroll
   for (int u = 0; u < U; u++)
      r[u] = t + NT * u < n ? __hip_atomic_load(src + t + NT * u, __ATOMIC_RELAXED, __HIP_MEMORY_SCOPE_AGENT) : T(0);
#pragma unroll
   for (int u = 0; u < U; u++)
      if (t + NT * u < 64 * N)
         dst[t + NT * u] = r[u];
}

template <typename T, int N, int NT>
struct RowRegs
{
   static constexpr int U = (64 * N + NT - 1) / NT;
   T r[U];
   MH_DEV void issue(const T *src, int rows, int t = threadIdx.x)
   {
      const int last = rows * N - 1;
#pragma unroll
      for (int u = 0; u < U; u++)
         r[u] = src[t + NT * u < last ? t + NT * u : last];
   }
   MH_DEV void commit(lds_ptr<T> dst, int t = threadIdx.x) const
   {
#pragma unroll
      for (int u = 0; u < U; u++)
         if (t + NT * u < 64 * N)
            dst[t + NT * u] = r[u];
   }
};
#ifndef MH_ZV_TWO_STAGE
#define MH_ZV_TWO_STAGE 1
#endif
template <class TP>
struct ZvCols
{
   static constexpr int NV = Tree<TP>::total_dofs();
   static constexpr int body_of(int d)
   {
      for (int j = 0; j < TP::N; j++)
         if (d >= Tree<TP>::dof_ofs(j) && d < Tree<TP>::dof_ofs(j) + Tree<TP>::ndof(j))
            return j;
      return 0;
   }
   static constexpr bool trunk(int d) { return Split<TP>::is_trunk(body_of(d)); }
   static constexpr int aba_owner(int d) { return trunk(d) ? -1 : Split<TP>::owner(Split<TP>::limb_index_of_body(body_of(d))); }
   static constexpr int limb_number(int d)
   {
      int n = 0;
      for (int c = 0; c < d; c++)
         n += trunk(c) ? 0 : 1;
      return n;
   }
};
template <class TP, typename T, int OWNER>
struct ZvColRegs
{
   static constexpr int count()
   {
      int n = 0;
      for (int d = 0; d < ZvCols<TP>::NV; d++)
         n += ZvCols<TP>::aba_owner(d) == OWNER ? 1 : 0;
      return n;
   }
   T r[count() > 0 ? count() : 1];
   template <int D = 0, int K = 0>
   MH_DEV void issue(const T *src, int lane)
   {
      if constexpr (D < ZvCols<TP>::NV)
      {
         if constexpr (ZvCols<TP>::aba_owner(D) == OWNER)
         {
            r[K] = __hip_atomic_load(src + D * 64 + lane, __ATOMIC_RELAXED, __HIP_MEMORY_SCOPE_AGENT);
            issue<D + 1, K + 1>(src, lane);
         }
         else
            issue<D + 1, K>(src, lane);
      }
   }
   template <int D = 0, int K = 0>
   MH_DEV void commit(lds_ptr<T> row) const
   {
      if constexpr (D < ZvCols<TP>::NV)
      {
         if constexpr (ZvCols<TP>::aba_owner(D) == OWNER)
         {
            row[D] = r[K];
            commit<D + 1, K + 1>(row);
         }
         else
            commit<D + 1, K>(row);
      }
   }
   template <int D = 0>
   MH_DEV void reset(T *dst, int lane) const
   {
      if constexpr (D < ZvCols<TP>::NV && sizeof(T) == 8)
      {
         if constexpr (ZvCols<TP>::aba_owner(D) == OWNER)
            __hip_atomic_store(reinterpret_cast<unsigned long long *>(dst) + D * 64 + lane, 0x7ff4a5a57ff4a5a5ull, __ATOMIC_RELAXED, __HIP_MEMORY_SCOPE_AGENT);
         reset<D + 1>(dst, lane);
      }
   }
};
#ifndef MH_ZV_SELF_SIGNAL
#define MH_ZV_SELF_SIGNAL 1
#endif
constexpr unsigned long long ZV_SENTINEL = 0x7ff4a5a57ff4a5a5ull;
constexpr int ZV_POISON_WORD = 3;
template <typename T>
MH_DEV bool zv_is_sentinel(T v)
{
   if constexpr (sizeof(T) == 8)
      return __builtin_bit_cast(unsigned long long, v) == ZV_SENTINEL;
   else
      return false;
}
template <class TP, typename T, int OWNER>
MH_DEV bool zv_cols_pending(const ZvColRegs<TP, T, OWNER> &c)
{
   bool p = false;
#pragma unroll
   for (int i = 0; i < ZvColRegs<TP, T, OWNER>::count(); i++)
      p = p || zv_is_sentinel(c.r[i]);
   return p;
}
template <class TP, typename T, int OWNER>
MH_DEV bool zv_take_cols(const ZvSync &sy, const T *src, T *reset, lds_ptr<T> row, int lane, bool active, int poison)
{
   ZvColRegs<TP, T, OWNER> c;
   bool ok = poison == 0;
   if (ok)
   {
      c.issue(src, lane);
      if (__builtin_amdgcn_ballot_w64(active && zv_cols_pending(c)) != 0)
      {
         const unsigned long long t0 = __builtin_amdgcn_s_memrealtime();
         for (;;)
         {
            __builtin_amdgcn_s_sleep(1);
            c.issue(src, lane);
            if (__builtin_amdgcn_ballot_w64(active && zv_cols_pending(c)) == 0)
               break;
            if (__builtin_amdgcn_s_memrealtime() - t0 > (unsigned long long)sy.wait_ticks)
            {
               ok = false;
               break;
            }
         }
      }
   }
   if (ok)
   {
      c.commit(row);
      c.reset(reset, lane);
   }
   else if ((threadIdx.x & 63) == 0)
   {
      __hip_atomic_store(sy.error, 1, __ATOMIC_RELAXED, __HIP_MEMORY_SCOPE_SYSTEM);
      __hip_atomic_store(sy.error + 1, 1, __ATOMIC_RELAXED, __HIP_MEMORY_SCOPE_SYSTEM);
      __hip_atomic_store(sy.flags + ZV_POISON_WORD, 1, __ATOMIC_RELAXED, __HIP_MEMORY_SCOPE_AGENT);
   }
   return ok;
}
template <class TP, typename T, int SHARE>
struct ZvPublish
{
   static constexpr bool mine(int d) { return SHARE < 0 ? ZvCols<TP>::trunk(d) : (!ZvCols<TP>::trunk(d) && ZvCols<TP>::limb_number(d) % 3 == SHARE); }
   static constexpr int count()
   {
      int n = 0;
      for (int d = 0; d < ZvCols<TP>::NV; d++)
         n += mine(d) ? 1 : 0;
      return n;
   }
   T r[count() > 0 ? count() : 1];
   template <int D = 0, int K = 0>
   MH_DEV void read(lds_ptr<T> row)
   {
      if constexpr (D < ZvCols<TP>::NV)
      {
         if constexpr (mine(D))
         {
            r[K] = row[D];
            read<D + 1, K + 1>(row);
         }
         else
            read<D + 1, K>(row);
      }
   }
   template <int D = 0, int K = 0>
   MH_DEV void read_minus(lds_ptr<T> tau_row, lds_ptr<T> row)
   {
      if constexpr (D < ZvCols<TP>::NV)
      {
         if constexpr (mine(D))
         {
            r[K] = tau_row[D] - row[D];
            read_minus<D + 1, K + 1>(tau_row, row);
         }
         else
            read_minus<D + 1, K>(tau_row, row);
      }
   }
   template <int D = 0, int K = 0>
   MH_DEV void store(T *dst, int lane) const
   {
      if constexpr (D < ZvCols<TP>::NV)
      {
         if constexpr (mine(D))
         {
            __hip_atomic_store(dst + D * 64 + lane, r[K], __ATOMIC_RELAXED, __HIP_MEMORY_SCOPE_AGENT);
            store<D + 1, K + 1>(dst, lane);
         }
         else
            store<D + 1, K>(dst, lane);
      }
   }
   static MH_DEV void run(T *dst, lds_ptr<T> row, int lane)
   {
      ZvPublish p;
      p.read(row);
      p.store(dst, lane);
   }
   static MH_DEV void run_minus(T *dst, lds_ptr<T> tau_row, lds_ptr<T> row, int lane)
   {
      ZvPublish p;
      p.read_minus(tau_row, row);
      p.store(dst, lane);
   }
};
#ifndef MH_ZV_TAU_LATE
#define MH_ZV_TAU_LATE 0
#endif
template <class TP>
constexpr int zv_bias_extra_rows()
{
   return MH_ZV_TAU_LATE && MH_ZV_TWO_STAGE ? Tree<TP>::total_dofs() : 0;
}
template <class TP, typename T>
MH_DEV void zv_bias_group2(const Args<T> &A, long k, lds_ptr<T> lds, T *taup, const ZvSync &sy)
{
   using S = Split<TP>;
   using CX = Ctx<T, true, true, std::conditional_t<MH_RNEA_PRE != 0, RneaPreStore<TP>, SplitStore<TP>>, false, MH_ZV_TAU_LATE ? 0 : 1>;
   const int wave = __builtin_amdgcn_readfirstlane((int)(threadIdx.x >> 6));
   const int lane = threadIdx.x & 63;
   constexpr int nq = Tree<TP>::total_cfgs(), nv = Tree<TP>::total_dofs();
   const lds_ptr<T> lxc = lds, lst = lxc + S::n_limbs() * 6 * 64, lq = lst + S::RNEA_TRUNK_SLOTS * 64, lqd = lq + 64 * nq, lx = lqd + 64 * nv;
   const lds_ptr<T> lt = lx + 64 * nv;
   ZV_STAMP(0, 14);
   const long cfg0 = k * 64;
   const int rows = (int)(A.B - cfg0 < 64 ? A.B - cfg0 : 64);
   const bool active = lane < rows;
   __shared__ int zv_limb_waves;
   if (threadIdx.x == 0)
      zv_limb_waves = 0;
   ZV_STAMP(0, 0);
   RowRegs<T, MH_ZV_TAU_LATE ? Tree<TP>::total_dofs() : 1, 256> rtau;
   if constexpr (MH_ZV_TAU_LATE)
   {
      RowRegs<T, Tree<TP>::total_cfgs(), 256> rq;
      RowRegs<T, Tree<TP>::total_dofs(), 256> rd;
      rq.issue(A.q + cfg0 * nq, rows), rd.issue(A.qd + cfg0 * nv, rows), rtau.issue(A.in3 + cfg0 * nv, rows);
      rq.commit(lq), rd.commit(lqd);
      zv_lds_barrier();
   }
   else
   {
      wave_stage_in<T, Tree<TP>::total_cfgs(), Tree<TP>::total_dofs(), 256>(lq, lqd, lx, A.q + cfg0 * nq, A.qd + cfg0 * nv, A.in3 + cfg0 * nv, rows);
      __syncthreads();
   }
   CX cx;
   fill_ctx<T>(cx, A, active ? cfg0 + lane : cfg0);
   cx.coriolis = 1, cx.accel = 0;
   cx.lq = lq + lane * nq, cx.lqd = lqd + lane * nv, cx.lx = lx + lane * nv, cx.lo = cx.lx;
   cx.wave = wave;
   cx.xbase = lxc + lane;
   cx.st.lbase = lst + lane;
   cx.st.gbase = nullptr, cx.st.stride = 0, cx.st.lane = 0;
   ZV_STAMP(0, 1);
   if (active)
      split_rnea_limbs<TP, 0, T, CX>(cx);
   ZV_STAMP(0, 2);
   if constexpr (MH_ZV_TAU_LATE)
      rtau.commit(lt);
   __syncthreads();
   ZV_STAMP(0, 3);
   T *const dst = taup + k * 64 * nv;
   int *const flags = sy.flags + k * ZV_SYNC_STRIDE;
   if (wave == 0)
   {
      if (active)
         rnea_trunk_roots<TP, T, CX>(cx);
      ZV_STAMP(0, 4);
      if constexpr (MH_ZV_TAU_LATE)
         ZvPublish<TP, T, -1>::run_minus(dst, lt + lane * nv, lx + lane * nv, lane);
      else
         ZvPublish<TP, T, -1>::run(dst, lx + lane * nv, lane);
      ZV_STAMP(0, 5);
#ifdef MH_ZV_TEST_FLAG_BEFORE_DRAIN
      if (lane == 0)
         __hip_atomic_store(flags, sy.epoch, __ATOMIC_RELAXED, __HIP_MEMORY_SCOPE_AGENT);
#endif
      asm volatile("s_waitcnt vmcnt(0)" ::: "memory");
      ZV_STAMP(0, 6);
#if !defined(MH_ZV_TEST_FLAG_BEFORE_DRAIN) && !defined(MH_ZV_TEST_NO_FLAG)
      if (lane == 0)
         __hip_atomic_store(flags, sy.epoch, __ATOMIC_RELAXED, __HIP_MEMORY_SCOPE_AGENT);
#endif
      ZV_STAMP(0, 7);
   }
   else
   {
      ZV_STAMP(0, 4);
#if !(MH_ZV_SELF_SIGNAL && defined(MH_ZV_TEST_NO_FLAG))
      if constexpr (MH_ZV_TAU_LATE)
      {
         if (wave == 1)
            ZvPublish<TP, T, 0>::run_minus(dst, lt + lane * nv, lx + lane * nv, lane);
         else if (wave == 2)
            ZvPublish<TP, T, 1>::run_minus(dst, lt + lane * nv, lx + lane * nv, lane);
         else
            ZvPublish<TP, T, 2>::run_minus(dst, lt + lane * nv, lx + lane * nv, lane);
      }
      else if (wave == 1)
         ZvPublish<TP, T, 0>::run(dst, lx + lane * nv, lane);
      else if (wave == 2)
         ZvPublish<TP, T, 1>::run(dst, lx + lane * nv, lane);
      else
         ZvPublish<TP, T, 2>::run(dst, lx + lane * nv, lane);
#endif
      ZV_STAMP(0, 5);
#if !MH_ZV_SELF_SIGNAL
      asm volatile("s_waitcnt vmcnt(0)" ::: "memory");
      ZV_STAMP(0, 6);
      int before = 0;
      if (lane == 0)
         before = __hip_atomic_fetch_add(&zv_limb_waves, 1, __ATOMIC_RELAXED, __HIP_MEMORY_SCOPE_WORKGROUP);
#ifndef MH_ZV_TEST_NO_FLAG
      if (lane == 0 && before == 2)
         __hip_atomic_store(flags + 1, sy.epoch, __ATOMIC_RELAXED, __HIP_MEMORY_SCOPE_AGENT);
#endif
#endif
      ZV_STAMP(0, 7);
   }
}

template <class TP, typename T, bool IDENT>
MH_DEV void zv_bias_group(const Args<T> &A, long k, lds_ptr<T> lds, T *taup, const ZvSync &sy)
{
   using S = Split<TP>;
   using CX = Ctx<T, true, IDENT, std::conditional_t<MH_RNEA_PRE != 0, RneaPreStore<TP>, SplitStore<TP>>, false, 1>;
   const int wave = __builtin_amdgcn_readfirstlane((int)(threadIdx.x >> 6));
   const int lane = threadIdx.x & 63;
   const int nq = A.m.nq, nv = A.m.nv;
   const lds_ptr<T> lxc = lds, lst = lxc + S::n_limbs() * 6 * 64, lq = lst + S::RNEA_TRUNK_SLOTS * 64, lqd = lq + 64 * nq, lx = lqd + 64 * nv;
   ZV_STAMP(0, 14);
   const long cfg0 = k * 64;
   const int rows = (int)(A.B - cfg0 < 64 ? A.B - cfg0 : 64);
   const bool active = lane < rows;
   __shared__ int zv_same_l2;
   ZV_STAMP(0, 0);
   wave_stage_in<T, Tree<TP>::total_cfgs(), Tree<TP>::total_dofs(), 256>(lq, lqd, lx, A.q + cfg0 * nq, A.qd + cfg0 * nv, A.in3 + cfg0 * nv, rows);
   __syncthreads();
   ZV_STAMP(0, 1);
   CX cx;
   fill_ctx<T>(cx, A, active ? cfg0 + lane : cfg0);
   cx.coriolis = 1, cx.accel = 0;
   cx.lq = lq + lane * nq, cx.lqd = lqd + lane * nv, cx.lx = lx + lane * nv, cx.lo = cx.lx;
   cx.wave = wave;
   cx.xbase = lxc + lane;
   cx.st.lbase = lst + lane;
   cx.st.gbase = nullptr, cx.st.stride = 0, cx.st.lane = 0;
   if (active)
      split_rnea_limbs<TP, 0, T, CX>(cx);
   ZV_STAMP(0, 2);
   if (threadIdx.x == 64)
      zv_same_l2 = sy.same_l2 && __hip_atomic_load(sy.flags + k * ZV_SYNC_STRIDE + 32, __ATOMIC_RELAXED, __HIP_MEMORY_SCOPE_AGENT) == zv_mail_key(sy.epoch, zv_xcc_id());
   __syncthreads();
   ZV_STAMP(0, 3);
   const bool same = zv_same_l2 != 0;
   if (active && wave == 0)
      rnea_trunk_roots<TP, T, CX>(cx);
   ZV_STAMP(0, 4);
   __syncthreads();
   zv_publish_rows<T, 256>(taup + cfg0 * nv, lx, rows * nv, same);
   ZV_STAMP(0, 5);
#ifdef MH_ZV_TEST_FLAG_BEFORE_DRAIN
   if (threadIdx.x == 0)
      __hip_atomic_store(sy.flags + k * ZV_SYNC_STRIDE, sy.epoch, __ATOMIC_RELAXED, __HIP_MEMORY_SCOPE_AGENT);
#endif
   asm volatile("s_waitcnt vmcnt(0)" ::: "memory");
   ZV_STAMP(0, 6);
   __syncthreads();
#if !defined(MH_ZV_TEST_FLAG_BEFORE_DRAIN) && !defined(MH_ZV_TEST_NO_FLAG)
   if (threadIdx.x == 0)
   {
      if (same)
         __hip_atomic_store(sy.flags + k * ZV_SYNC_STRIDE, sy.epoch, __ATOMIC_RELAXED, __HIP_MEMORY_SCOPE_WORKGROUP);
      else
         __hip_atomic_store(sy.flags + k * ZV_SYNC_STRIDE, sy.epoch, __ATOMIC_RELAXED, __HIP_MEMORY_SCOPE_AGENT);
   }
#endif
   ZV_STAMP(0, 7);
}

template <class TP, typename T, bool IDENT>
MH_DEV void zv_aba_group(const Args<T> &A, long k, lds_ptr<T> lds, const T *taup, const ZvSync &sy)
{
   using S = Split<TP>;
#ifndef MH_ZV_DIRECT_OUT
#define MH_ZV_DIRECT_OUT 0
#endif
   using CX = Ctx<T, true, IDENT, ZvStore<TP>, false, MH_ZV_DIRECT_OUT ? 2 : 0>;
   const int wave = __builtin_amdgcn_readfirstlane((int)(threadIdx.x >> 6));
   const int lane = threadIdx.x & 63;
   const int nq = A.m.nq, nv = A.m.nv;
   const lds_ptr<T> lxc = lds, lst = lxc + S::n_limbs() * ZV_XW * 64, lq = lst + S::ZV_TRUNK_SLOTS * 64, lx = lq + 64 * nq, lres = lx + 64 * nv;
   ZV_STAMP(1, 14);
   const long cfg0 = k * 64;
   const int rows = (int)(A.B - cfg0 < 64 ? A.B - cfg0 : 64);
   const bool active = lane < rows;
   ZV_STAMP(1, 0);
   if (sy.same_l2 && threadIdx.x == 0)
      __hip_atomic_store(sy.flags + k * ZV_SYNC_STRIDE + 32, zv_mail_key(sy.epoch, zv_xcc_id()), __ATOMIC_RELAXED, __HIP_MEMORY_SCOPE_AGENT);
   zv_stage_rows<T, Tree<TP>::total_cfgs(), 256>(lq, A.q + cfg0 * nq, rows);
   __syncthreads();
   ZV_STAMP(1, 1);
   CX cx;
   fill_ctx<T>(cx, A, active ? cfg0 + lane : cfg0);
   cx.lq = lq + lane * nq, cx.lqd = lq, cx.lx = lx + lane * nv, cx.lo = lres + lane * nv;
   cx.wave = wave;
   cx.xbase = lxc + lane;
   cx.st.lbase = lst + lane;
   cx.st.gbase = nullptr, cx.st.stride = 0, cx.st.lane = 0;
#ifdef MH_ZV_PROBE
   cx.own = (unsigned long long)k;
#endif
#ifdef MH_ZV_TWICE
#pragma unroll 1
   for (int rep = 0; rep < 2; rep++)
   {
      asm volatile("" ::: "memory");
      if (active)
         zv_limbs_in<TP, 0, T, CX>(cx);
      if (rep == 0)
      {
         ZV_STAMP(1, 12);
         __syncthreads();
         ZV_STAMP(1, 13);
      }
   }
#else
   if (active)
      zv_limbs_in<TP, 0, T, CX>(cx);
#endif
   ZV_STAMP(1, 2);
   __syncthreads();
   ZV_STAMP(1, 3);
   if (active)
      zv_roots_in<TP, T, CX, (S::staged() ? 2 : 1)>(cx);
   ZV_STAMP(1, 4);
   __shared__ int zv_gave_up;
   if (wave == 0)
   {
      const bool seen = zv_wait(sy, k);
      if (lane == 0)
         zv_gave_up = seen ? 0 : 1;
   }
   __syncthreads();
   if (zv_gave_up)
   {
      for (int i = threadIdx.x; i < rows * nv; i += 256)
      {
         if constexpr (sizeof(T) == 8)
            reinterpret_cast<unsigned long long *>(A.out)[cfg0 * nv + i] = 0x7ff8000000000000ull;
         else
            reinterpret_cast<unsigned *>(A.out)[cfg0 * nv + i] = 0x7fc00000u;
      }
      return;
   }
   ZV_STAMP(1, 5);
   zv_fetch_rows<T, Tree<TP>::total_dofs(), 256>(lx, taup + cfg0 * nv, rows);
   if (threadIdx.x == 0)
   {
      __hip_atomic_store(sy.flags + k * ZV_SYNC_STRIDE, 0, __ATOMIC_RELAXED, __HIP_MEMORY_SCOPE_AGENT);
      if (sy.same_l2)
         __hip_atomic_store(sy.flags + k * ZV_SYNC_STRIDE + 32, 0, __ATOMIC_RELAXED, __HIP_MEMORY_SCOPE_AGENT);
   }
   __syncthreads();
   ZV_STAMP(1, 6);
   asm volatile("" ::: "memory");
   if (active)
      zv_fold_out<TP, 0, T, CX>(cx);
   ZV_STAMP(1, 10);
   if constexpr (!MH_ZV_DIRECT_OUT)
   {
      __syncthreads();
      wave_copy_out<T, 256>(A.out + cfg0 * nv, lres, rows * nv);
   }
   ZV_STAMP(1, 11);
}

MH_DEV bool zv_wait_word(const ZvSync &sy, const int *f)
{
   if (__hip_atomic_load(f, __ATOMIC_RELAXED, __HIP_MEMORY_SCOPE_AGENT) == sy.epoch)
      return true;
   const unsigned long long t0 = __builtin_amdgcn_s_memrealtime();
   for (;;)
   {
      __builtin_amdgcn_s_sleep(1);
      if (__hip_atomic_load(f, __ATOMIC_RELAXED, __HIP_MEMORY_SCOPE_AGENT) == sy.epoch)
         return true;
      if (__builtin_amdgcn_s_memrealtime() - t0 > (unsigned long long)sy.wait_ticks)
      {
         if ((threadIdx.x & 63) == 0)
            __hip_atomic_store(sy.error, 1, __ATOMIC_RELAXED, __HIP_MEMORY_SCOPE_SYSTEM);
         return false;
      }
   }
}
template <class TP, typename T, bool STEP>
MH_DEV void zv_aba_group2(const Args<T> &A, long k, lds_ptr<T> lds, const T *taup, const ZvSync &sy)
{
   using S = Split<TP>;
   using CX = Ctx<T, true, true, ZvStore<TP>, false, 0>;
   const int wave = __builtin_amdgcn_readfirstlane((int)(threadIdx.x >> 6));
   const int lane = threadIdx.x & 63;
   constexpr int nq = Tree<TP>::total_cfgs(), nv = Tree<TP>::total_dofs();
   const lds_ptr<T> lxc = lds, lst = lxc + S::n_limbs() * ZV_XW * 64, lq = lst + S::ZV_TRUNK_SLOTS * 64, lx = lq + 64 * nq, lres = lx + 64 * nv;
   ZV_STAMP(1, 14);
   const long cfg0 = k * 64;
   const int rows = (int)(A.B - cfg0 < 64 ? A.B - cfg0 : 64);
   const bool active = lane < rows;
   __shared__ int zv_gave_up;
   if (threadIdx.x == 0)
      zv_gave_up = 0;
   ZV_STAMP(1, 0);
#if MH_ZV_SELF_SIGNAL
   const int poison = __hip_atomic_load(sy.flags + ZV_POISON_WORD, __ATOMIC_RELAXED, __HIP_MEMORY_SCOPE_AGENT);
#endif
   zv_stage_rows<T, Tree<TP>::total_cfgs(), 256>(lq, A.q + cfg0 * nq, rows);
   __syncthreads();
   ZV_STAMP(1, 1);
   CX cx;
   fill_ctx<T>(cx, A, active ? cfg0 + lane : cfg0);
   cx.lq = lq + lane * nq, cx.lqd = lq, cx.lx = lx + lane * nv, cx.lo = lres + lane * nv;
   cx.wave = wave;
   cx.xbase = lxc + lane;
   cx.st.lbase = lst + lane;
   cx.st.gbase = nullptr, cx.st.stride = 0, cx.st.lane = 0;
#ifdef MH_ZV_PROBE
   cx.own = (unsigned long long)k;
#endif
   if (active)
      zv_limbs_in<TP, 0, T, CX>(cx);
   ZV_STAMP(1, 2);
   __syncthreads();
   ZV_STAMP(1, 3);
   if (active)
      zv_roots_in<TP, T, CX, (S::staged() ? 2 : 1)>(cx);
   ZV_STAMP(1, 4);
   RowRegs<T, STEP ? Tree<TP>::total_dofs() : 1, 256> rqd;
   if constexpr (STEP)
      rqd.issue(A.qd + cfg0 * nv, rows);
   const T *const src = taup + k * 64 * nv;
   const int *const flags = sy.flags + k * ZV_SYNC_STRIDE;
   const lds_ptr<T> row = lx + lane * nv;
#if MH_ZV_SELF_SIGNAL
   bool seen;
   {
      T *const back = const_cast<T *>(src);
      if (wave == 0)
         seen = zv_take_cols<TP, T, 0>(sy, src, back, row, lane, active, poison);
      else if (wave == 1)
         seen = zv_take_cols<TP, T, 1>(sy, src, back, row, lane, active, poison);
      else if (wave == 2)
         seen = zv_take_cols<TP, T, 2>(sy, src, back, row, lane, active, poison);
      else
         seen = zv_take_cols<TP, T, 3>(sy, src, back, row, lane, active, poison);
   }
   ZV_STAMP(1, 5);
#else
   bool seen = zv_wait_word(sy, flags + 1);
   ZV_STAMP(1, 5);
   if (wave == 0)
   {
      ZvColRegs<TP, T, 0> c;
      c.issue(src, lane), c.commit(row);
   }
   else if (wave == 1)
   {
      ZvColRegs<TP, T, 1> c;
      c.issue(src, lane), c.commit(row);
   }
   else if (wave == 2)
   {
      ZvColRegs<TP, T, 2> c;
      c.issue(src, lane), c.commit(row);
   }
   else
   {
      ZvColRegs<TP, T, 3> c;
      c.issue(src, lane), c.commit(row);
   }
#endif
   const int b_first = __hip_atomic_load(flags, __ATOMIC_RELAXED, __HIP_MEMORY_SCOPE_AGENT);
   zv_lds_barrier();
   ZV_STAMP(1, 6);
   asm volatile("" ::: "memory");
   struct TrunkTau : ZvNoHook
   {
      mutable ZvColRegs<TP, T, -1> c;
      const ZvSync &sy;
      const int *flags;
      const T *src;
      lds_ptr<T> row;
      int lane, b_first;
      bool &seen;
      MH_DEV void after_early() const
      {
         if (b_first != sy.epoch)
            seen = zv_wait_word(sy, flags) && seen;
         c.issue(src, lane);
      }
      MH_DEV void after_late() const { c.commit(row); }
   };
   const TrunkTau trunk{{}, {}, sy, flags, src, row, lane, b_first, seen};
   if (active)
      zv_fold_out<TP, 0, T, CX>(cx, trunk);
   ZV_STAMP(1, 10);
   if (!seen && lane == 0)
      zv_gave_up = 1;
   __syncthreads();
   if (threadIdx.x == 0)
   {
      __hip_atomic_store(const_cast<int *>(flags), 0, __ATOMIC_RELAXED, __HIP_MEMORY_SCOPE_AGENT);
      __hip_atomic_store(const_cast<int *>(flags) + 1, 0, __ATOMIC_RELAXED, __HIP_MEMORY_SCOPE_AGENT);
   }
   if (zv_gave_up)
   {
      for (int i = threadIdx.x; i < rows * nv; i += 256)
         reinterpret_cast<unsigned long long *>(A.out)[cfg0 * nv + i] = 0x7ff8000000000000ull;
      if constexpr (STEP)
      {
         for (int i = threadIdx.x; i < rows * nq; i += 256)
            reinterpret_cast<unsigned long long *>(A.q_next)[cfg0 * nq + i] = 0x7ff8000000000000ull;
         for (int i = threadIdx.x; i < rows * nv; i += 256)
            reinterpret_cast<unsigned long long *>(A.qd_next)[cfg0 * nv + i] = 0x7ff8000000000000ull;
      }
      return;
   }
   if constexpr (STEP)
   {
      rqd.commit(lx);
      __syncthreads();
      if (active)
         integrate_rows<TP, 0, T>(wave, lq + lane * nq, lx + lane * nv, lres + lane * nv, A.dt, T(0.5) * A.dt * A.dt);
      __syncthreads();
      wave_copy_out<T, 256>(A.q_next + cfg0 * nq, lq, rows * nq);
      wave_copy_out<T, 256>(A.qd_next + cfg0 * nv, lx, rows * nv);
   }
   wave_copy_out<T, 256>(A.out + cfg0 * nv, lres, rows * nv);
   ZV_STAMP(1, 11);
}

#ifndef MH_ZV_KERNEL_ATTR
#define MH_ZV_KERNEL_ATTR
#endif
template <class TP, typename T, bool IDENT, bool STEP = false>
__global__ void __launch_bounds__(256) MH_ZV_KERNEL_ATTR spec_zv_kernel(const T *q0, const T *qd0, const T *tau0, long B0, int jobs0, Args<T> A_full, T *taup,
                                                                        ZvSync sy_full)
{
   extern __shared__ double lds_raw[];
   const int blk = (int)blockIdx.x;
   Args<T> A = A_full;
   A.q = q0, A.qd = qd0, A.in3b = tau0, A.B = B0;
   ZvSync sy = sy_full;
   sy.jobs = jobs0;
   const int padded = (int)gridDim.x / sy.jobs;
   const bool tail = sy.jobs == 3 && blk >= 2 * padded;
   const int role = tail ? 2 : (blk >> 3) & 1;
   const long k = tail ? (long)(blk - 2 * padded) : (long)(blk / 16) * 8 + (blk & 7);
   if (k * 64 >= A.B)
      return;
   ZV_STAMP(role, 15);
   if (role == 0)
   {
      Args<T> A2 = A;
      A2.in3 = A.in3b;
      if constexpr (IDENT && MH_ZV_TWO_STAGE && sizeof(T) == 8)
         zv_bias_group2<TP, T>(A2, k, (lds_ptr<T>)lds_raw, taup, sy);
      else
         zv_bias_group<TP, T, IDENT>(A2, k, (lds_ptr<T>)lds_raw, taup, sy);
   }
   else if (role == 1)
   {
      Args<T> A2 = A;
      A2.out = A.outb;
      if constexpr (IDENT && MH_ZV_TWO_STAGE && sizeof(T) == 8)
         zv_aba_group2<TP, T, STEP>(A2, k, (lds_ptr<T>)lds_raw, taup, sy);
      else
         zv_aba_group<TP, T, IDENT>(A2, k, (lds_ptr<T>)lds_raw, taup, sy);
   }
   else
   {
      split_group<TP, T, 0, IDENT, true>(A, k, (A.B + 63) / 64, (lds_ptr<T>)lds_raw);
      ZV_STAMP(2, 1);
   }
}

template <class TP>
struct ZvbPlan
{
   using S = Split<TP>;
   static constexpr int NV = Tree<TP>::total_dofs();
   static constexpr int x_slots()
   {
      const int in = S::n_limbs() * ZV_XW, fold = NV + S::n_limbs() * 12;
      return in > fold ? in : fold;
   }
   static constexpr int lds_slots() { return x_slots() + ZvbStore<TP>::TRUNK_SLOTS; }
   static constexpr int bias_lds_slots(int nq, int nv) { return S::n_limbs() * 6 + S::RNEA_TRUNK_SLOTS + nq + 2 * nv; }
};


template <class TP, typename T, bool IDENT, bool BIAS = true>
__global__ void __launch_bounds__(256, 2) spec_zvb_bias_kernel(Args<T> A, T *taup, T *cs, long cs_stride)
{
   extern __shared__ double lds_raw[];
   using S = Split<TP>;
   using CX = Ctx<T, true, IDENT, std::conditional_t<MH_RNEA_PRE != 0, RneaPreStore<TP>, SplitStore<TP>>, false, BIAS ? 1 : 0, BIAS ? 1 : 0>;
   constexpr int NQ = Tree<TP>::total_cfgs(), NV = Tree<TP>::total_dofs();
   const lds_ptr<T> lds = (lds_ptr<T>)lds_raw;
   const int wave = __builtin_amdgcn_readfirstlane((int)(threadIdx.x >> 6));
   const int lane = threadIdx.x & 63;
   const int nq = A.m.nq, nv = A.m.nv;
   const lds_ptr<T> lxc = lds, lst = lxc + S::n_limbs() * 6 * 64, lq = lst + S::RNEA_TRUNK_SLOTS * 64, lqd = lq + 64 * nq, lx = lqd + 64 * nv;
   RowRegs<T, NQ, 192> rq;
   RowRegs<T, NV, 192> rd, rx;
   const int loader = (int)threadIdx.x - 64;
   auto request = [&](long k) {
      const long cfg0 = k * 64;
      const int rows = (int)(A.B - cfg0 < 64 ? A.B - cfg0 : 64);
      rq.issue(A.q + cfg0 * nq, rows, loader), rd.issue(A.qd + cfg0 * nv, rows, loader), rx.issue(A.in3 + cfg0 * nv, rows, loader);
   };
   const long ngroups = (A.B + 63) / 64;
   if (wave != 0)
      request(blockIdx.x);
   for (long k = blockIdx.x; k < ngroups; k += gridDim.x)
   {
      const long cfg0 = k * 64;
      const int rows = (int)(A.B - cfg0 < 64 ? A.B - cfg0 : 64);
      const bool active = lane < rows;
      ZV_STAMP(0, 0);
      if (wave != 0)
         rq.commit(lq, loader), rd.commit(lqd, loader), rx.commit(lx, loader);
      __syncthreads();
      ZV_STAMP(0, 1);
      CX cx;
      fill_ctx<T>(cx, A, active ? cfg0 + lane : cfg0);
      if constexpr (BIAS)
         cx.coriolis = 1, cx.accel = 0;
      cx.lq = lq + lane * nq, cx.lqd = lqd + lane * nv, cx.lx = lx + lane * nv, cx.lo = cx.lx;
      cx.wave = wave;
      cx.xbase = lxc + lane;
      cx.st.lbase = lst + lane;
      cx.st.gbase = nullptr, cx.st.stride = 0, cx.st.lane = 0;
      if constexpr (BIAS)
         cx.cs = cs + cfg0 + lane, cx.cs_stride = cs_stride;
      if (active)
         split_rnea_limbs<TP, 0, T, CX>(cx);
      ZV_STAMP(0, 2);
      __syncthreads();
      ZV_STAMP(0, 3);
      if (wave != 0)
         request(k + gridDim.x < ngroups ? k + gridDim.x : k);
      else if (active)
         rnea_trunk_roots<TP, T, CX>(cx);
      ZV_STAMP(0, 4);
      zv_lds_barrier();
      wave_copy_out<T, 256>(taup + cfg0 * nv, lx, rows * nv);
      ZV_STAMP(0, 5);
      zv_lds_barrier();
      ZV_STAMP(0, 6);
   }
}

template <class TP, typename T, bool IDENT>
MH_DEV void zvb_aba_group(const Args<T> &A, long k, lds_ptr<T> lds, const T *taup, const T *cs, long cs_stride)
{
   using S = Split<TP>;
   using PL = ZvbPlan<TP>;
   using CX = Ctx<T, true, IDENT, ZvbStore<TP>, false, 0, 2>;
   const int wave = __builtin_amdgcn_readfirstlane((int)(threadIdx.x >> 6));
   const int lane = threadIdx.x & 63;
   const int nv = A.m.nv;
   const lds_ptr<T> lxc = lds, lst = lxc + PL::x_slots() * 64, lx = lxc, lfold = lxc + 64 * nv;
   const long cfg0 = k * 64;
   const int rows = (int)(A.B - cfg0 < 64 ? A.B - cfg0 : 64);
   const bool active = lane < rows;
   CX cx;
   fill_ctx<T>(cx, A, active ? cfg0 + lane : cfg0);
   cx.lq = lxc, cx.lqd = lxc;
   cx.lx = lx + lane * nv, cx.lo = cx.lx;
   cx.wave = wave;
   cx.xbase = lxc + lane;
   cx.st.lbase = lst + lane;
   cx.st.gbase = nullptr, cx.st.stride = 0, cx.st.lane = 0;
   cx.cs = const_cast<T *>(cs) + cfg0 + lane, cx.cs_stride = cs_stride;
#ifdef MH_ZV_PROBE
   cx.own = (unsigned long long)k;
#endif
   ZV_STAMP(1, 0);
   if (active)
      zv_limbs_in<TP, 0, T, CX>(cx);
   ZV_STAMP(1, 2);
   __syncthreads();
   ZV_STAMP(1, 3);
// ... 328 lines not shown
```

Before: 304.6 million configs/s.

## Publish per-body RNEA wrenches as self-signalling sentinel columns for ABA consumer

```diff
diff --git a/mecano_amd/csrc/mh_api.hip b/mecano_amd/csrc/mh_api.hip
--- a/mecano_amd/csrc/mh_api.hip
+++ b/mecano_amd/csrc/mh_api.hip
@@ -508,16 +508,17 @@
       return fail(MH_ERR_HIP, "a bias-split forward dynamics launch gave up waiting for its bias rows (the accelerations of those configurations were written as NaN)");
    return MH_OK;
 }
-bool zv_self_signalling(const mh_model *m) { return m->ident_maps && m->spec.zv_self_signal && m->spec.zv_self_signal() != 0; }
+bool zv_self_signalling(const mh_model *m) { return m->ident_maps && m->spec.zv_self_signal && m->spec.zv_self_signal() > 0; }
 mh_status zv_prepare(mh_model *m, int64_t B, hipStream_t stream)
 {
    const size_t groups = (size_t)groups_of(B);
    mh_status st = ensure_bytes(m->zv_tau, groups * 64 * m->nv * sizeof(double));
    if (st != MH_OK)
       return st;
-   if (zv_self_signalling(m) && m->zv_cols.bytes < groups * 64 * m->nv * sizeof(double))
-   {
-      st = ensure_bytes(m->zv_cols, std::max<size_t>(groups, 128) * 64 * m->nv * sizeof(double));
+   const size_t cols = zv_self_signalling(m) ? (size_t)m->spec.zv_self_signal() : 0;
+   if (cols > 0 && m->zv_cols.bytes < groups * 64 * cols * sizeof(double))
+   {
+      st = ensure_bytes(m->zv_cols, std::max<size_t>(groups, 128) * 64 * cols * sizeof(double));
       if (st != MH_OK)
          return st;
       HIP_TRY(hipMemsetD32Async((hipDeviceptr_t)m->zv_cols.ptr, 0x7ff4a5a5, m->zv_cols.bytes / 4, stream));
diff --git a/mecano_amd/csrc/mh_spec.hip b/mecano_amd/csrc/mh_spec.hip
--- a/mecano_amd/csrc/mh_spec.hip
+++ b/mecano_amd/csrc/mh_spec.hip
@@ -249,11 +249,11 @@
 {
    if constexpr (!SPL::usable())
       return 0;
-   const long inertia = (long)(SPL::n_limbs() * mh::ZV_XW + SPL::ZV_TRUNK_SLOTS + nq + 2 * nv) * 64 * (long)sizeof(double);
-   return std::max(inertia, split_lds_bytes(0, F_IO_LDS, nq, nv) + (long)mh::zv_bias_extra_rows<TP>() * 64 * (long)sizeof(double));
+   const long inertia = (long)(SPL::n_limbs() * mh::ZV_XW + mh::ZvwStore<TP>::TRUNK_SLOTS + nq + 2 * nv) * 64 * (long)sizeof(double);
+   return std::max(inertia, split_lds_bytes(0, F_IO_LDS, nq, nv));
 }
 int mh_spec_zv_usable(void) { return SPL::usable() ? 1 : 0; }
-int mh_spec_zv_self_signal(void) { return MH_ZV_TWO_STAGE && MH_ZV_SELF_SIGNAL ? 1 : 0; }
+int mh_spec_zv_self_signal(void) { return MH_ZV_TWO_STAGE ? mh::ZvCols<TP>::NC : 0; }
 #ifdef MH_ZV_PROBE
 int mh_spec_zv_probe_read(void *dst, size_t bytes) { return (int)hipMemcpyFromSymbol(dst, HIP_SYMBOL(mh::zv_probe), bytes); }
 int mh_spec_zv_probe_body_read(void *dst, size_t bytes) { return (int)hipMemcpyFromSymbol(dst, HIP_SYMBOL(mh::zv_probe_body), bytes); }
@@ -291,7 +291,7 @@
          hipLaunchKernelGGL(kern, dim3((unsigned)(padded * jobs)), dim3(256), lds, s, A.q, A.qd, A.in3b, A.B, jobs, A, (double *)taup, sy);
          return (int)hipGetLastError();
       }
-#ifdef MH_SPEC_MINIMAL
+#if defined(MH_SPEC_MINIMAL) && !defined(MH_ZV_TEST_FLAG_BEFORE_DRAIN)
       return (int)hipErrorNotSupported;
 #else
       static LdsAttr attr2;
diff --git a/mecano_amd/csrc/mh_spec_kernels.h b/mecano_amd/csrc/mh_spec_kernels.h
--- a/mecano_amd/csrc/mh_spec_kernels.h
+++ b/mecano_amd/csrc/mh_spec_kernels.h
@@ -817,9 +817,31 @@
                 V3<T>{x_get<LIMB, XW, I0 + 3, CX, T>(cx), x_get<LIMB, XW, I0 + 4, CX, T>(cx), x_get<LIMB, XW, I0 + 5, CX, T>(cx)}};
 }
 
+template <int J, class CX, typename T>
+MH_DEV void wrench_cols_put(const CX &cx, const SV<T> &w)
+{
+#ifndef MH_ZV_TEST_NO_FLAG
+   T *const d = cx.cs + 6 * J * 64;
+   __hip_atomic_store(d + 0 * 64, w.a.x, __ATOMIC_RELAXED, __HIP_MEMORY_SCOPE_AGENT);
+   __hip_atomic_store(d + 1 * 64, w.a.y, __ATOMIC_RELAXED, __HIP_MEMORY_SCOPE_AGENT);
+   __hip_atomic_store(d + 2 * 64, w.a.z, __ATOMIC_RELAXED, __HIP_MEMORY_SCOPE_AGENT);
+   __hip_atomic_store(d + 3 * 64, w.l.x, __ATOMIC_RELAXED, __HIP_MEMORY_SCOPE_AGENT);
+   __hip_atomic_store(d + 4 * 64, w.l.y, __ATOMIC_RELAXED, __HIP_MEMORY_SCOPE_AGENT);
+   __hip_atomic_store(d + 5 * 64, w.l.z, __ATOMIC_RELAXED, __HIP_MEMORY_SCOPE_AGENT);
+#endif
+}
 template <class TP, int J, typename T, class CX, int MODE = 0>
 struct RneaSub
 {
+   template <int K>
+   static MH_DEV void children_out(const CX &cx, const SV<T> &v, const SV<T> &a)
+   {
+      if constexpr (K < Tree<TP>::n_children(J))
+      {
+         (void)RneaSub<TP, Tree<TP>::child(J, K), T, CX, MODE>::run(cx, v, a);
+         children_out<K + 1>(cx, v, a);
+      }
+   }
    template <int K>
    static MH_DEV void children(const CX &cx, const SV<T> &v, const SV<T> &a, SV<T> &f)
    {
@@ -875,6 +897,12 @@
       if (cx.frow)
          f = f - load_fext<T>(c, cx.frow, cx.f_es, cx.meta[J * MI_STRIDE + MI_EXT]);
       MH_BODY_FENCE();
+      if constexpr (CX::csmode == 4)
+      {
+         wrench_cols_put<J, CX, T>(cx, f);
+         children_out<0>(cx, v, a);
+         return SV<T>{Z, Z};
+      }
       children<0>(cx, v, a, f);
       MH_BODY_FENCE();
       if constexpr (CX::csmode == 3)
@@ -941,11 +969,16 @@
       SV<T> f = mul(I, a) + crf(v, mul(I, v));
       if (cx.frow)
          f = f - load_fext<T>(c, cx.frow, cx.f_es, cx.meta[J * MI_STRIDE + MI_EXT]);
-      constexpr int S0 = Split<TP>::rnea_trunk_slot(J);
-      const lds_ptr<T> t = rnea_park<CX, T>(cx);
-      t[(S0 + 0) * 64] = f.a.x, t[(S0 + 1) * 64] = f.a.y, t[(S0 + 2) * 64] = f.a.z;
-      t[(S0 + 3) * 64] = f.l.x, t[(S0 + 4) * 64] = f.l.y, t[(S0 + 5) * 64] = f.l.z;
-      t[(S0 + 6) * 64] = jx.c, t[(S0 + 7) * 64] = jx.s;
+      if constexpr (CX::csmode == 4)
+         wrench_cols_put<J, CX, T>(cx, f);
+      else
+      {
+         constexpr int S0 = Split<TP>::rnea_trunk_slot(J);
+         const lds_ptr<T> t = rnea_park<CX, T>(cx);
+         t[(S0 + 0) * 64] = f.a.x, t[(S0 + 1) * 64] = f.a.y, t[(S0 + 2) * 64] = f.a.z;
+         t[(S0 + 3) * 64] = f.l.x, t[(S0 + 4) * 64] = f.l.y, t[(S0 + 5) * 64] = f.l.z;
+         t[(S0 + 6) * 64] = jx.c, t[(S0 + 7) * 64] = jx.s;
+      }
       if constexpr (CX::csmode == 1 && TYPE == JT_REVOLUTE)
       {
          constexpr int R = Tree<TP>::rev_index(J);
@@ -2124,7 +2157,10 @@
             if constexpr (P >= 0)
                trunk_va<TP, P, T, CX, K, OWN>(cx, vp, ap);
          }
-         x_put6<K, 6, 0, CX, T>(cx, RneaSub<TP, R, T, CX, 0>::run(cx, vp, ap));
+         if constexpr (CX::csmode == 4)
+            (void)RneaSub<TP, R, T, CX, 0>::run(cx, vp, ap);
+         else
+            x_put6<K, 6, 0, CX, T>(cx, RneaSub<TP, R, T, CX, 0>::run(cx, vp, ap));
          split_rnea_limbs_of<TP, W, K + 1, P, T, CX, OWN>(cx, vp, ap);
       }
       else
diff --git a/mecano_amd/csrc/mh_zv_kernels.h b/mecano_amd/csrc/mh_zv_kernels.h
--- a/mecano_amd/csrc/mh_zv_kernels.h
+++ b/mecano_amd/csrc/mh_zv_kernels.h
@@ -10,6 +10,62 @@
    static constexpr int kind(int j) { return Split<TP>::is_trunk(j) ? ST_LDS_KIND : ST_REG_KIND; }
    static constexpr int index(int j) { return Split<TP>::is_trunk(j) ? Split<TP>::zv_trunk_slot(j) : Split<TP>::zv_reg_slot(j); }
    static constexpr bool shared(int j) { return !Split<TP>::is_trunk(j); }
+};
+template <class TP>
+struct ZvwStore
+{
+   using S = Split<TP>;
+   static constexpr bool slot_homes = true;
+   static constexpr bool wrench_slots = true;
+   static constexpr int wrench_slot(int j) { return Tree<TP>::zv_slots_of(j, !S::is_trunk(j)); }
+   static constexpr int rank(int j)
+   {
+      int n = 0;
+      for (int i = 0; i < j; i++)
+         n += S::is_trunk(j) ? (S::is_trunk(i) ? 1 : 0) : (!S::is_trunk(i) && S::owner(S::limb_index_of_body(i)) == S::owner(S::limb_index_of_body(j)) ? 1 : 0);
+      return n;
+   }
+   static constexpr int limb_bodies()
+   {
+      int best = 0;
+      for (int w = 0; w < 4; w++)
+      {
+         int n = 0;
+         for (int j = 0; j < TP::N; j++)
+            n += !S::is_trunk(j) && S::owner(S::limb_index_of_body(j)) == w ? 1 : 0;
+         best = n > best ? n : best;
+      }
+      return best;
+   }
+   static constexpr int trunk_bodies()
+   {
+      int n = 0;
+      for (int j = 0; j < TP::N; j++)
+         n += S::is_trunk(j) ? 1 : 0;
+      return n;
+   }
+   static constexpr int REG_SLOTS = S::zv_reg_slots() + 6 * limb_bodies();
+   static constexpr int TRUNK_SLOTS = S::ZV_TRUNK_SLOTS + 6 * trunk_bodies();
+   static constexpr int kind(int j) { return ZvStore<TP>::kind(j); }
+   static constexpr int index(int j) { return ZvStore<TP>::index(j); }
+   static constexpr bool shared(int j) { return ZvStore<TP>::shared(j); }
+   static constexpr int slot_kind(int j, int) { return kind(j); }
+   static constexpr int slot_index(int j, int k)
+   {
+      if (k < wrench_slot(j))
+         return index(j) + k;
+      return (S::is_trunk(j) ? S::ZV_TRUNK_SLOTS : S::zv_reg_slots()) + 6 * rank(j) + (k - wrench_slot(j));
+   }
+};
+template <class SP, class = void>
+struct policy_wrench_slots
+{
+   static constexpr bool value = false;
+};
+template <class SP>
+struct policy_wrench_slots<SP, std::enable_if_t<SP::wrench_slots>>
+{
+   static constexpr bool value = true;
 };
 template <class TP>
 struct ZvbStore
@@ -429,6 +485,7 @@
 template <class TP, int J, typename T, class CX, int MODE = 0>
 struct ZvFold
 {
+   static constexpr bool SEED = policy_wrench_slots<typename CX::SPolicy>::value;
    template <int K>
    static MH_DEV void children(const CX &cx, SV<T> &pA)
    {
@@ -442,7 +499,7 @@
             c = x_get6<Split<TP>::sub_slot(C), CX::fold_xw, 6, CX, T>(cx);
          else
             c = ZvFold<TP, C, T, CX, MODE>::run(cx);
-         if constexpr (K == 0)
+         if constexpr (K == 0 && !SEED)
             pA = c;
          else
             pA = pA + c;
@@ -459,6 +516,12 @@
       constexpr int RS = Tree<TP>::zv_result_slot(J, CX::SPolicy::shared(J));
       const V3<T> Z{T(0), T(0), T(0)};
       SV<T> pA{Z, Z};
+      if constexpr (SEED)
+      {
+         constexpr int W0 = CX::SPolicy::wrench_slot(J);
+         pA = SV<T>{V3<T>{cx.st.template get<J, W0 + 0>(), cx.st.template get<J, W0 + 1>(), cx.st.template get<J, W0 + 2>()},
+                    V3<T>{cx.st.template get<J, W0 + 3>(), cx.st.template get<J, W0 + 4>(), cx.st.template get<J, W0 + 5>()}};
+      }
       if constexpr (!LEAF)
          children<0>(cx, pA);
       MH_BODY_FENCE();
@@ -988,44 +1051,59 @@
 #ifndef MH_ZV_TWO_STAGE
 #define MH_ZV_TWO_STAGE 1
 #endif
+constexpr unsigned long long ZV_SENTINEL = 0x7ff4a5a57ff4a5a5ull;
+constexpr int ZV_POISON_WORD = 3;
+template <typename T>
+MH_DEV bool zv_is_sentinel(T v)
+{
+   if constexpr (sizeof(T) == 8)
+      return __builtin_bit_cast(unsigned long long, v) == ZV_SENTINEL;
+   else
+      return false;
+}
 template <class TP>
 struct ZvCols
 {
+   using S = Split<TP>;
    static constexpr int NV = Tree<TP>::total_dofs();
-   static constexpr int body_of(int d)
+   static constexpr int NW = 6 * TP::N;
+   static constexpr int NC = NW + NV;
+   static constexpr int dof_body(int d)
    {
       for (int j = 0; j < TP::N; j++)
          if (d >= Tree<TP>::dof_ofs(j) && d < Tree<TP>::dof_ofs(j) + Tree<TP>::ndof(j))
             return j;
       return 0;
    }
-   static constexpr bool trunk(int d) { return Split<TP>::is_trunk(body_of(d)); }
-   static constexpr int aba_owner(int d) { return trunk(d) ? -1 : Split<TP>::owner(Split<TP>::limb_index_of_body(body_of(d))); }
-   static constexpr int limb_number(int d)
+   static constexpr int body_of(int c) { return c < NW ? c / 6 : dof_body(c - NW); }
+   static constexpr bool trunk(int c) { return S::is_trunk(body_of(c)); }
+   static constexpr int aba_owner(int c) { return trunk(c) ? -1 : S::owner(S::limb_index_of_body(body_of(c))); }
+   static constexpr int limb_dof_number(int d)
    {
       int n = 0;
-      for (int c = 0; c < d; c++)
-         n += trunk(c) ? 0 : 1;
+      for (int e = 0; e < d; e++)
+         n += trunk(NW + e) ? 0 : 1;
       return n;
    }
 };
 template <class TP, typename T, int OWNER>
 struct ZvColRegs
 {
+   using C = ZvCols<TP>;
    static constexpr int count()
    {
       int n = 0;
-      for (int d = 0; d < ZvCols<TP>::NV; d++)
-         n += ZvCols<TP>::aba_owner(d) == OWNER ? 1 : 0;
+      for (int c = 0; c < C::NC; c++)
+         n += C::aba_owner(c) == OWNER ? 1 : 0;
       return n;
    }
    T r[count() > 0 ? count() : 1];
    template <int D = 0, int K = 0>
    MH_DEV void issue(const T *src, int lane)
    {
-      if constexpr (D < ZvCols<TP>::NV)
-      {
-         if constexpr (ZvCols<TP>::aba_owner(D) == OWNER)
+      if constexpr (D < C::NC)
+      {
+         if constexpr (C::aba_owner(D) == OWNER)
          {
             r[K] = __hip_atomic_load(src + D * 64 + lane, __ATOMIC_RELAXED, __HIP_MEMORY_SCOPE_AGENT);
             issue<D + 1, K + 1>(src, lane);
@@ -1034,69 +1112,64 @@
             issue<D + 1, K>(src, lane);
       }
    }
-   template <int D = 0, int K = 0>
-   MH_DEV void commit(lds_ptr<T> row) const
-   {
-      if constexpr (D < ZvCols<TP>::NV)
-      {
-         if constexpr (ZvCols<TP>::aba_owner(D) == OWNER)
+   template <int I = 0>
+   MH_DEV bool pending() const
+   {
+      if constexpr (I < count())
+         return zv_is_sentinel(r[I]) | pending<I + 1>();
+      else
+         return false;
+   }
+   template <class SP, int D = 0, int K = 0>
+   MH_DEV void commit(T *regs, lds_ptr<T> lbase, lds_ptr<T> row) const
+   {
+      if constexpr (D < C::NC)
+      {
+         if constexpr (C::aba_owner(D) == OWNER)
          {
-            row[D] = r[K];
-            commit<D + 1, K + 1>(row);
+            if constexpr (D < C::NW)
+            {
+               constexpr int slot = SP::slot_index(D / 6, SP::wrench_slot(D / 6) + D % 6);
+               if constexpr (SP::kind(D / 6) == ST_LDS_KIND)
+                  lbase[slot * 64] = r[K];
+               else
+                  regs[slot] = r[K];
+            }
+            else
+               row[D - C::NW] = r[K];
+            commit<SP, D + 1, K + 1>(regs, lbase, row);
          }
          else
-            commit<D + 1, K>(row);
+            commit<SP, D + 1, K>(regs, lbase, row);
       }
    }
    template <int D = 0>
-   MH_DEV void reset(T *dst, int lane) const
-   {
-      if constexpr (D < ZvCols<TP>::NV && sizeof(T) == 8)
-      {
-         if constexpr (ZvCols<TP>::aba_owner(D) == OWNER)
-            __hip_atomic_store(reinterpret_cast<unsigned long long *>(dst) + D * 64 + lane, 0x7ff4a5a57ff4a5a5ull, __ATOMIC_RELAXED, __HIP_MEMORY_SCOPE_AGENT);
+   static MH_DEV void reset(T *dst, int lane)
+   {
+      if constexpr (D < C::NC && sizeof(T) == 8)
+      {
+         if constexpr (C::aba_owner(D) == OWNER)
+            __hip_atomic_store(reinterpret_cast<unsigned long long *>(dst) + D * 64 + lane, ZV_SENTINEL, __ATOMIC_RELAXED, __HIP_MEMORY_SCOPE_AGENT);
          reset<D + 1>(dst, lane);
       }
    }
 };
-#ifndef MH_ZV_SELF_SIGNAL
-#define MH_ZV_SELF_SIGNAL 1
-#endif
-constexpr unsigned long long ZV_SENTINEL = 0x7ff4a5a57ff4a5a5ull;
-constexpr int ZV_POISON_WORD = 3;
-template <typename T>
-MH_DEV bool zv_is_sentinel(T v)
-{
-   if constexpr (sizeof(T) == 8)
-      return __builtin_bit_cast(unsigned long long, v) == ZV_SENTINEL;
-   else
-      return false;
-}
 template <class TP, typename T, int OWNER>
-MH_DEV bool zv_cols_pending(const ZvColRegs<TP, T, OWNER> &c)
-{
-   bool p = false;
-#pragma unroll
-   for (int i = 0; i < ZvColRegs<TP, T, OWNER>::count(); i++)
-      p = p || zv_is_sentinel(c.r[i]);
-   return p;
-}
-template <class TP, typename T, int OWNER>
-MH_DEV bool zv_take_cols(const ZvSync &sy, const T *src, T *reset, lds_ptr<T> row, int lane, bool active, int poison)
-{
-   ZvColRegs<TP, T, OWNER> c;
+MH_DEV bool zv_poll_cols(const ZvSync &sy, ZvColRegs<TP, T, OWNER> &c, const T *src, int lane, bool active, int poison, bool issued)
+{
    bool ok = poison == 0;
    if (ok)
    {
-      c.issue(src, lane);
-      if (__builtin_amdgcn_ballot_w64(active && zv_cols_pending(c)) != 0)
+      if (!issued)
+         c.issue(src, lane);
+      if (__builtin_amdgcn_ballot_w64(active && c.pending()) != 0)
       {
          const unsigned long long t0 = __builtin_amdgcn_s_memrealtime();
          for (;;)
          {
             __builtin_amdgcn_s_sleep(1);
             c.issue(src, lane);
-            if (__builtin_amdgcn_ballot_w64(active && zv_cols_pending(c)) == 0)
+            if (__builtin_amdgcn_ballot_w64(active && c.pending()) == 0)
                break;
             if (__builtin_amdgcn_s_memrealtime() - t0 > (unsigned long long)sy.wait_ticks)
             {
@@ -1106,12 +1179,7 @@
          }
       }
    }
-   if (ok)
-   {
-      c.commit(row);
-      c.reset(reset, lane);
-   }
-   else if ((threadIdx.x & 63) == 0)
+   if (!ok && (threadIdx.x & 63) == 0)
    {
       __hip_atomic_store(sy.error, 1, __ATOMIC_RELAXED, __HIP_MEMORY_SCOPE_SYSTEM);
       __hip_atomic_store(sy.error + 1, 1, __ATOMIC_RELAXED, __HIP_MEMORY_SCOPE_SYSTEM);
@@ -1119,14 +1187,27 @@
    }
    return ok;
 }
+template <class TP, typename T, int OWNER, class CX>
+MH_DEV bool zv_take_cols(const ZvSync &sy, const CX &cx, const T *src, T *reset, lds_ptr<T> row, int lane, bool active, int poison)
+{
+   ZvColRegs<TP, T, OWNER> c;
+   const bool ok = zv_poll_cols<TP, T, OWNER>(sy, c, src, lane, active, poison, false);
+   if (ok)
+   {
+      c.template commit<typename CX::SPolicy>(cx.st.regs, cx.st.lbase, row);
+      c.reset(reset, lane);
+   }
+   return ok;
+}
 template <class TP, typename T, int SHARE>
 struct ZvPublish
 {
-   static constexpr bool mine(int d) { return SHARE < 0 ? ZvCols<TP>::trunk(d) : (!ZvCols<TP>::trunk(d) && ZvCols<TP>::limb_number(d) % 3 == SHARE); }
+   using C = ZvCols<TP>;
+   static constexpr bool mine(int d) { return SHARE < 0 ? C::trunk(C::NW + d) : (!C::trunk(C::NW + d) && C::limb_dof_number(d) % 3 == SHARE); }
    static constexpr int count()
    {
       int n = 0;
-      for (int d = 0; d < ZvCols<TP>::NV; d++)
+      for (int d = 0; d < C::NV; d++)
          n += mine(d) ? 1 : 0;
       return n;
    }
@@ -1134,7 +1215,7 @@
    template <int D = 0, int K = 0>
    MH_DEV void read(lds_ptr<T> row)
    {
-      if constexpr (D < ZvCols<TP>::NV)
+      if constexpr (D < C::NV)
       {
          if constexpr (mine(D))
          {
@@ -1146,27 +1227,13 @@
       }
    }
    template <int D = 0, int K = 0>
-   MH_DEV void read_minus(lds_ptr<T> tau_row, lds_ptr<T> row)
-   {
-      if constexpr (D < ZvCols<TP>::NV)
+   MH_DEV void store(T *dst, int lane) const
+   {
+      if constexpr (D < C::NV)
       {
          if constexpr (mine(D))
          {
-            r[K] = tau_row[D] - row[D];
-            read_minus<D + 1, K + 1>(tau_row, row);
-         }
-         else
-            read_minus<D + 1, K>(tau_row, row);
-      }
-   }
-   template <int D = 0, int K = 0>
-   MH_DEV void store(T *dst, int lane) const
-   {
-      if constexpr (D < ZvCols<TP>::NV)
-      {
-         if constexpr (mine(D))
-         {
-            __hip_atomic_store(dst + D * 64 + lane, r[K], __ATOMIC_RELAXED, __HIP_MEMORY_SCOPE_AGENT);
+            __hip_atomic_store(dst + (C::NW + D) * 64 + lane, r[K], __ATOMIC_RELAXED, __HIP_MEMORY_SCOPE_AGENT);
             store<D + 1, K + 1>(dst, lane);
          }
          else
@@ -1179,53 +1246,24 @@
       p.read(row);
       p.store(dst, lane);
    }
-   static MH_DEV void run_minus(T *dst, lds_ptr<T> tau_row, lds_ptr<T> row, int lane)
-   {
-      ZvPublish p;
-      p.read_minus(tau_row, row);
-      p.store(dst, lane);
-   }
-};
-#ifndef MH_ZV_TAU_LATE
-#define MH_ZV_TAU_LATE 0
-#endif
-template <class TP>
-constexpr int zv_bias_extra_rows()
-{
-   return MH_ZV_TAU_LATE && MH_ZV_TWO_STAGE ? Tree<TP>::total_dofs() : 0;
-}
+};
 template <class TP, typename T>
-MH_DEV void zv_bias_group2(const Args<T> &A, long k, lds_ptr<T> lds, T *taup, const ZvSync &sy)
-{
-   using S = Split<TP>;
-   using CX = Ctx<T, true, true, std::conditional_t<MH_RNEA_PRE != 0, RneaPreStore<TP>, SplitStore<TP>>, false, MH_ZV_TAU_LATE ? 0 : 1>;
+MH_DEV void zv_bias_group2(const Args<T> &A, long k, lds_ptr<T> lds, T *cols, const ZvSync &sy)
+{
+   using S = Split<TP>;
+   using CX = Ctx<T, true, true, std::conditional_t<MH_RNEA_PRE != 0, RneaPreStore<TP>, SplitStore<TP>>, false, 0, 4>;
    const int wave = __builtin_amdgcn_readfirstlane((int)(threadIdx.x >> 6));
    const int lane = threadIdx.x & 63;
    constexpr int nq = Tree<TP>::total_cfgs(), nv = Tree<TP>::total_dofs();
    const lds_ptr<T> lxc = lds, lst = lxc + S::n_limbs() * 6 * 64, lq = lst + S::RNEA_TRUNK_SLOTS * 64, lqd = lq + 64 * nq, lx = lqd + 64 * nv;
-   const lds_ptr<T> lt = lx + 64 * nv;
    ZV_STAMP(0, 14);
    const long cfg0 = k * 64;
    const int rows = (int)(A.B - cfg0 < 64 ? A.B - cfg0 : 64);
    const bool active = lane < rows;
-   __shared__ int zv_limb_waves;
-   if (threadIdx.x == 0)
-      zv_limb_waves = 0;
    ZV_STAMP(0, 0);
-   RowRegs<T, MH_ZV_TAU_LATE ? Tree<TP>::total_dofs() : 1, 256> rtau;
-   if constexpr (MH_ZV_TAU_LATE)
-   {
-      RowRegs<T, Tree<TP>::total_cfgs(), 256> rq;
-      RowRegs<T, Tree<TP>::total_dofs(), 256> rd;
-      rq.issue(A.q + cfg0 * nq, rows), rd.issue(A.qd + cfg0 * nv, rows), rtau.issue(A.in3 + cfg0 * nv, rows);
-      rq.commit(lq), rd.commit(lqd);
-      zv_lds_barrier();
-   }
-   else
-   {
-      wave_stage_in<T, Tree<TP>::total_cfgs(), Tree<TP>::total_dofs(), 256>(lq, lqd, lx, A.q + cfg0 * nq, A.qd + cfg0 * nv, A.in3 + cfg0 * nv, rows);
-      __syncthreads();
-   }
+   wave_stage_in<T, Tree<TP>::total_cfgs(), Tree<TP>::total_dofs(), 256>(lq, lqd, lx, A.q + cfg0 * nq, A.qd + cfg0 * nv, A.in3 + cfg0 * nv, rows);
+   __syncthreads();
+   T *const dst = cols + k * 64 * ZvCols<TP>::NC;
    CX cx;
    fill_ctx<T>(cx, A, active ? cfg0 + lane : cfg0);
    cx.coriolis = 1, cx.accel = 0;
@@ -1234,74 +1272,23 @@
    cx.xbase = lxc + lane;
    cx.st.lbase = lst + lane;
    cx.st.gbase = nullptr, cx.st.stride = 0, cx.st.lane = 0;
+   cx.cs = dst + lane, cx.cs_stride = 0;
    ZV_STAMP(0, 1);
    if (active)
       split_rnea_limbs<TP, 0, T, CX>(cx);
    ZV_STAMP(0, 2);
-   if constexpr (MH_ZV_TAU_LATE)
-      rtau.commit(lt);
-   __syncthreads();
-   ZV_STAMP(0, 3);
-   T *const dst = taup + k * 64 * nv;
-   int *const flags = sy.flags + k * ZV_SYNC_STRIDE;
+#ifndef MH_ZV_TEST_NO_FLAG
    if (wave == 0)
-   {
-      if (active)
-         rnea_trunk_roots<TP, T, CX>(cx);
-      ZV_STAMP(0, 4);
-      if constexpr (MH_ZV_TAU_LATE)
-         ZvPublish<TP, T, -1>::run_minus(dst, lt + lane * nv, lx + lane * nv, lane);
-      else
-         ZvPublish<TP, T, -1>::run(dst, lx + lane * nv, lane);
-      ZV_STAMP(0, 5);
-#ifdef MH_ZV_TEST_FLAG_BEFORE_DRAIN
-      if (lane == 0)
-         __hip_atomic_store(flags, sy.epoch, __ATOMIC_RELAXED, __HIP_MEMORY_SCOPE_AGENT);
+      ZvPublish<TP, T, -1>::run(dst, lx + lane * nv, lane);
+   else if (wave == 1)
+      ZvPublish<TP, T, 0>::run(dst, lx + lane * nv, lane);
+   else if (wave == 2)
+      ZvPublish<TP, T, 1>::run(dst, lx + lane * nv, lane);
+   else
+      ZvPublish<TP, T, 2>::run(dst, lx + lane * nv, lane);
 #endif
-      asm volatile("s_waitcnt vmcnt(0)" ::: "memory");
-      ZV_STAMP(0, 6);
-#if !defined(MH_ZV_TEST_FLAG_BEFORE_DRAIN) && !defined(MH_ZV_TEST_NO_FLAG)
-      if (lane == 0)
-         __hip_atomic_store(flags, sy.epoch, __ATOMIC_RELAXED, __HIP_MEMORY_SCOPE_AGENT);
-#endif
-      ZV_STAMP(0, 7);
-   }
-   else
-   {
-      ZV_STAMP(0, 4);
-#if !(MH_ZV_SELF_SIGNAL && defined(MH_ZV_TEST_NO_FLAG))
-      if constexpr (MH_ZV_TAU_LATE)
-      {
-         if (wave == 1)
-            ZvPublish<TP, T, 0>::run_minus(dst, lt + lane * nv, lx + lane * nv, lane);
-         else if (wave == 2)
-            ZvPublish<TP, T, 1>::run_minus(dst, lt + lane * nv, lx + lane * nv, lane);
-         else
-            ZvPublish<TP, T, 2>::run_minus(dst, lt + lane * nv, lx + lane * nv, lane);
-      }
-      else if (wave == 1)
-         ZvPublish<TP, T, 0>::run(dst, lx + lane * nv, lane);
-      else if (wave == 2)
-         ZvPublish<TP, T, 1>::run(dst, lx + lane * nv, lane);
-      else
-         ZvPublish<TP, T, 2>::run(dst, lx + lane * nv, lane);
-#endif
-      ZV_STAMP(0, 5);
-#if !MH_ZV_SELF_SIGNAL
-      asm volatile("s_waitcnt vmcnt(0)" ::: "memory");
-      ZV_STAMP(0, 6);
-      int before = 0;
-      if (lane == 0)
-         before = __hip_atomic_fetch_add(&zv_limb_waves, 1, __ATOMIC_RELAXED, __HIP_MEMORY_SCOPE_WORKGROUP);
-#ifndef MH_ZV_TEST_NO_FLAG
-      if (lane == 0 && before == 2)
-         __hip_atomic_store(flags + 1, sy.epoch, __ATOMIC_RELAXED, __HIP_MEMORY_SCOPE_AGENT);
-#endif
-#endif
-      ZV_STAMP(0, 7);
-   }
-}
-
+   ZV_STAMP(0, 5);
+}
 template <class TP, typename T, bool IDENT>
 MH_DEV void zv_bias_group(const Args<T> &A, long k, lds_ptr<T> lds, T *taup, const ZvSync &sy)
 {
@@ -1458,33 +1445,15 @@
    ZV_STAMP(1, 11);
 }
 
-MH_DEV bool zv_wait_word(const ZvSync &sy, const int *f)
-{
-   if (__hip_atomic_load(f, __ATOMIC_RELAXED, __HIP_MEMORY_SCOPE_AGENT) == sy.epoch)
-      return true;
-   const unsigned long long t0 = __builtin_amdgcn_s_memrealtime();
-   for (;;)
-   {
-      __builtin_amdgcn_s_sleep(1);
-      if (__hip_atomic_load(f, __ATOMIC_RELAXED, __HIP_MEMORY_SCOPE_AGENT) == sy.epoch)
-         return true;
-      if (__builtin_amdgcn_s_memrealtime() - t0 > (unsigned long long)sy.wait_ticks)
-      {
-         if ((threadIdx.x & 63) == 0)
-            __hip_atomic_store(sy.error, 1, __ATOMIC_RELAXED, __HIP_MEMORY_SCOPE_SYSTEM);
-         return false;
-      }
-   }
-}
 template <class TP, typename T, bool STEP>
-MH_DEV void zv_aba_group2(const Args<T> &A, long k, lds_ptr<T> lds, const T *taup, const ZvSync &sy)
-{
-   using S = Split<TP>;
-   using CX = Ctx<T, true, true, ZvStore<TP>, false, 0>;
+MH_DEV void zv_aba_group2(const Args<T> &A, long k, lds_ptr<T> lds, const T *cols, const ZvSync &sy)
+{
+   using S = Split<TP>;
+   using CX = Ctx<T, true, true, ZvwStore<TP>, false, 0>;
    const int wave = __builtin_amdgcn_readfirstlane((int)(threadIdx.x >> 6));
    const int lane = threadIdx.x & 63;
    constexpr int nq = Tree<TP>::total_cfgs(), nv = Tree<TP>::total_dofs();
-   const lds_ptr<T> lxc = lds, lst = lxc + S::n_limbs() * ZV_XW * 64, lq = lst + S::ZV_TRUNK_SLOTS * 64, lx = lq + 64 * nq, lres = lx + 64 * nv;
+   const lds_ptr<T> lxc = lds, lst = lxc + S::n_limbs() * ZV_XW * 64, lq = lst + ZvwStore<TP>::TRUNK_SLOTS * 64, lx = lq + 64 * nq, lres = lx + 64 * nv;
    ZV_STAMP(1, 14);
    const long cfg0 = k * 64;
    const int rows = (int)(A.B - cfg0 < 64 ? A.B - cfg0 : 64);
@@ -1493,9 +1462,7 @@
    if (threadIdx.x == 0)
       zv_gave_up = 0;
    ZV_STAMP(1, 0);
-#if MH_ZV_SELF_SIGNAL
    const int poison = __hip_atomic_load(sy.flags + ZV_POISON_WORD, __ATOMIC_RELAXED, __HIP_MEMORY_SCOPE_AGENT);
-#endif
    zv_stage_rows<T, Tree<TP>::total_cfgs(), 256>(lq, A.q + cfg0 * nq, rows);
    __syncthreads();
    ZV_STAMP(1, 1);
@@ -1520,80 +1487,48 @@
    RowRegs<T, STEP ? Tree<TP>::total_dofs() : 1, 256> rqd;
    if constexpr (STEP)
       rqd.issue(A.qd + cfg0 * nv, rows);
-   const T *const src = taup + k * 64 * nv;
-   const int *const flags = sy.flags + k * ZV_SYNC_STRIDE;
+   const T *const src = cols + k * 64 * ZvCols<TP>::NC;
+   T *const back = const_cast<T *>(src);
    const lds_ptr<T> row = lx + lane * nv;
-#if MH_ZV_SELF_SIGNAL
    bool seen;
-   {
-      T *const back = const_cast<T *>(src);
-      if (wave == 0)
-         seen = zv_take_cols<TP, T, 0>(sy, src, back, row, lane, active, poison);
-      else if (wave == 1)
-         seen = zv_take_cols<TP, T, 1>(sy, src, back, row, lane, active, poison);
-      else if (wave == 2)
-         seen = zv_take_cols<TP, T, 2>(sy, src, back, row, lane, active, poison);
-      else
-         seen = zv_take_cols<TP, T, 3>(sy, src, back, row, lane, active, poison);
-   }
+   if (wave == 0)
+      seen = zv_take_cols<TP, T, 0, CX>(sy, cx, src, back, row, lane, active, poison);
+   else if (wave == 1)
+      seen = zv_take_cols<TP, T, 1, CX>(sy, cx, src, back, row, lane, active, poison);
+   else if (wave == 2)
+      seen = zv_take_cols<TP, T, 2, CX>(sy, cx, src, back, row, lane, active, poison);
+   else
+      seen = zv_take_cols<TP, T, 3, CX>(sy, cx, src, back, row, lane, active, poison);
    ZV_STAMP(1, 5);
-#else
-   bool seen = zv_wait_word(sy, flags + 1);
-   ZV_STAMP(1, 5);
-   if (wave == 0)
-   {
-      ZvColRegs<TP, T, 0> c;
-      c.issue(src, lane), c.commit(row);
-   }
-   else if (wave == 1)
-   {
-      ZvColRegs<TP, T, 1> c;
-      c.issue(src, lane), c.commit(row);
-   }
-   else if (wave == 2)
-   {
-      ZvColRegs<TP, T, 2> c;
-      c.issue(src, lane), c.commit(row);
-   }
-   else
-   {
-      ZvColRegs<TP, T, 3> c;
-      c.issue(src, lane), c.commit(row);
-   }
-#endif
-   const int b_first = __hip_atomic_load(flags, __ATOMIC_RELAXED, __HIP_MEMORY_SCOPE_AGENT);
+   struct TrunkCols : ZvNoHook
+   {
+      mutable ZvColRegs<TP, T, -1> c;
+      const ZvSync &sy;
+      lds_ptr<T> lbase;
+      const T *src;
+      lds_ptr<T> row;
+      int lane, poison;
+      bool active;
+      bool &seen;
+      MH_DEV void after_early() const
+      {
+         seen = zv_poll_cols<TP, T, -1>(sy, c, src, lane, active, poison, true) && seen;
+         c.template commit<ZvwStore<TP>>(nullptr, lbase, row);
+      }
+   };
+   const TrunkCols trunk{{}, {}, sy, cx.st.lbase, src, row, lane, poison, active, seen};
+   trunk.c.issue(src, lane);
    zv_lds_barrier();
    ZV_STAMP(1, 6);
    asm volatile("" ::: "memory");
-   struct TrunkTau : ZvNoHook
-   {
-      mutable ZvColRegs<TP, T, -1> c;
-      const ZvSync &sy;
-      const int *flags;
-      const T *src;
-      lds_ptr<T> row;
-      int lane, b_first;
-      bool &seen;
-      MH_DEV void after_early() const
-      {
-         if (b_first != sy.epoch)
-            seen = zv_wait_word(sy, flags) && seen;
-         c.issue(src, lane);
-      }
-      MH_DEV void after_late() const { c.commit(row); }
-   };
-   const TrunkTau trunk{{}, {}, sy, flags, src, row, lane, b_first, seen};
    if (active)
       zv_fold_out<TP, 0, T, CX>(cx, trunk);
    ZV_STAMP(1, 10);
    if (!seen && lane == 0)
       zv_gave_up = 1;
    __syncthreads();
-   if (threadIdx.x == 0)
-   {
-      __hip_atomic_store(const_cast<int *>(flags), 0, __ATOMIC_RELAXED, __HIP_MEMORY_SCOPE_AGENT);
-      __hip_atomic_store(const_cast<int *>(flags) + 1, 0, __ATOMIC_RELAXED, __HIP_MEMORY_SCOPE_AGENT);
-   }
+   if (wave == 0 && !zv_gave_up)
+      ZvColRegs<TP, T, -1>::reset(back, lane);
    if (zv_gave_up)
    {
       for (int i = threadIdx.x; i < rows * nv; i += 256)
@@ -1620,7 +1555,6 @@
    wave_copy_out<T, 256>(A.out + cfg0 * nv, lres, rows * nv);
    ZV_STAMP(1, 11);
 }
-
 #ifndef MH_ZV_KERNEL_ATTR
 #define MH_ZV_KERNEL_ATTR
 #endif
```

New measurement: 77.33 million configs/s. -74.6%, worse.
